# AI4Science-WestlakeU/wdno

Measured on AMD Instinct MI355X. Metric: diffusion train steps/sec, 2D smoke U-Net (8 samples per GPU per step), higher is better.
Workload: dtype f32

## Files before the change

include/wdno_hip.h:

```cpp
#ifndef WDNO_HIP_H
#define WDNO_HIP_H
#include <stdint.h>
#include <stddef.h>

#ifdef __cplusplus
extern "C" {
#endif

typedef void* wdno_stream_t;

enum { WDNO_OK = 0, WDNO_EINVAL = -1, WDNO_ELAUNCH = -2, WDNO_EUNSUPPORTED = -3, WDNO_EWORKSPACE = -4 };

#define WDNO_AMAX_SLOTS 64
#define WDNO_AMAX_STRIDE 16
#define WDNO_AMAX_FLOATS (WDNO_AMAX_SLOTS * WDNO_AMAX_STRIDE)
const char* wdno_strerror(int code);
int wdno_version(void);
const char* wdno_last_hip_error(void);
int wdno_set_debug(int mode);

typedef struct {
  int nd;
  int mode;
  int L;
  int n_img;
  int in_dims[3];
  int out_dims[3];
  int64_t cs_img, cs_band, cs0, cs1;
} wdno_dwt_desc;
size_t wdno_dwt_ws_bytes(const wdno_dwt_desc* d);
int wdno_dwt_fwd(const float* x, float* coef, const wdno_dwt_desc* d, const float* filters_host, void* ws, size_t ws_bytes, wdno_stream_t s);
int wdno_dwt_inv(const float* coef, float* x, const wdno_dwt_desc* d, const float* filters_host, void* ws, size_t ws_bytes, wdno_stream_t s);
int wdno_dwt_fwd_adjoint(const float* dcoef, float* dx, const wdno_dwt_desc* d, const float* filters_host, void* ws, size_t ws_bytes, wdno_stream_t s);
int wdno_dwt_inv_adjoint(const float* dx, float* dcoef, const wdno_dwt_desc* d, const float* filters_host, void* ws, size_t ws_bytes, wdno_stream_t s);
int wdno_dwt_fwd_packed(const float* x, float* state, const wdno_dwt_desc* d, const float* filters_host, int img_inner, int64_t cs_outer, int row_w,
                        const float* rescaler, wdno_stream_t s);
int wdno_upsample_coef(const float* in, float* out, int64_t outer, int a, int mid, int b, int c, int fa, int fb, int fc, wdno_stream_t s);
int wdno_pack_smoke_state(const float* coef, int64_t coef_sim_stride, const float* init_coef, int64_t init_sim_stride, const float* smokeout,
                          int64_t so_sim_stride, const int64_t* idx, const float* rescaler, float* state, int64_t B, int F, int nt, int nx,
                          int pad_t, int pad_x, wdno_stream_t s);
int wdno_pack_smoke_fields(const float* coef, int64_t coef_sim_stride, const float* rho0, int64_t rho0_sim_stride, const float* curve,
                           int64_t curve_sim_stride, const float* dec_lo_host, const float* dec_hi_host, int L, const float* rescaler,
                           float* state, int64_t B, int F, int nt, int nx, int pad_t, int pad_x, int H0, int W0, int T0, wdno_stream_t s);

int wdno_nc_to_cl(const float* src, float* dst, int64_t N, int C, int64_t S, int Cp, wdno_stream_t s);
int wdno_cl_to_nc(const float* src, float* dst, int64_t N, int C, int64_t S, int Cp, wdno_stream_t s);
int wdno_concat2_cl_planes(const float* a, int Ca, const float* b, int Cb, const float* rec_a, const float* rec_b, void* hi, void* lo,
                           float* scale_out, int64_t P, wdno_stream_t s);
int wdno_concat2_cl(const float* a, int Ca, const float* b, int Cb, float* out, int64_t P, wdno_stream_t s);
int wdno_concat2_cl_amax(const float* a, int Ca, const float* b, int Cb, float* out, float* amax_rec, int64_t P, wdno_stream_t s);
int wdno_split2_cl(const float* in, float* a, int Ca, float* b, int Cb, int64_t P, wdno_stream_t s);
int wdno_upsample2x_cl_fwd(const float* in, float* out, int64_t N, int H, int W, int C, wdno_stream_t s);
int wdno_upsample2x_cl_bwd(const float* dout, float* din, int64_t N, int H, int W, int C, wdno_stream_t s);

typedef struct {
  int N, D, H, W, C;
  int OD, OH, OW, K;
  int kd, kh, kw;
  int sd, sh, sw;
  int pd, ph, pw;
  int YD, YH, YW;
  int osd, osh, osw, ood, ooh, oow;
} wdno_conv_geom;
int wdno_conv_fwd(const float* x, const float* wp, const float* bias, const float* residual, float* y,
                  const wdno_conv_geom* g, wdno_stream_t s);
int wdno_amax(const float* x, int64_t n, float* amax_zeroed, wdno_stream_t s);
int wdno_amax_record(const float* x, int64_t n, float* rec_zeroed, wdno_stream_t s);
int wdno_split_f16(const float* x, const float* amax_rec, void* hi, void* lo, float* scale_out, int64_t rows, int C, int C8, wdno_stream_t s);
size_t wdno_split_colsum_ws_bytes(int64_t rows, int C8);
int wdno_split_f16_colsum(const float* x, const float* amax_rec, void* hi, void* lo, float* scale_out, float* colsum_out,
                          void* ws, size_t ws_bytes, int64_t rows, int C, int C8, wdno_stream_t s);
int wdno_pack_split_weight(const float* w, const float* amax, void* hi, void* lo, float* scale_out, int K, int C, int kd, int kh, int kw,
                           int A, int B, int mode, wdno_stream_t s);
typedef struct { const void* x; int64_t n; void* out; } wdno_amax_item;
typedef struct {
  const void* w; const void* amax; void* hi; void* lo; void* scale_out;
  int K, C, kd, kh, kw, A, B, mode;
} wdno_wsplit_item;
int wdno_amax_multi(const void* table, int n_items, int blocks_per_item, wdno_stream_t s);
int wdno_pack_split_weight_multi(const void* table, int n_items, int blocks_per_item, wdno_stream_t s);
int wdno_conv_fwd_f16x3(const void* xh, const void* xl, const float* sx, const void* wph, const void* wpl, const float* sw,
                        const float* bias, const float* residual, float* y, const wdno_conv_geom* g, wdno_stream_t s);
int wdno_conv_fwd_f16x3_amax(const void* xh, const void* xl, const float* sx, const void* wph, const void* wpl, const float* sw,
                             const float* bias, const float* residual, float* y, float* amax_rec, const wdno_conv_geom* g,
                             wdno_stream_t s);
typedef struct { int channels, d0, h0, w0; } wdno_zero_box;
int wdno_conv_fwd_f16x3_zbox(const void* xh, const void* xl, const float* sx, const void* wph, const void* wpl, const float* sw,
                             const float* bias, const float* residual, float* y, float* amax_rec, const wdno_conv_geom* g,
                             const wdno_zero_box* zb, wdno_stream_t s);
int wdno_conv_fwd_bf16_ex(const void* x16, const void* wp16, const float* bias, const float* residual, void* y, int y_bf16, float* amax_rec,
                          const wdno_conv_geom* g, const wdno_zero_box* zb, wdno_stream_t s);
int wdno_conv_fwd_f16x3_ws(const void* xh, const void* xl, const float* sx, const void* wph, const void* wpl, const float* sw,
                           const float* bias, const float* residual, float* y, float* amax_rec, const wdno_conv_geom* g,
                           void* ws, size_t ws_bytes, wdno_stream_t s);
size_t wdno_conv_fwd_split_ws_bytes(const wdno_conv_geom* g);
size_t wdno_conv_wgrad_f16x3_ws_bytes(const wdno_conv_geom* g);
int wdno_conv_pixel_table(void* table, const wdno_conv_geom* g, wdno_stream_t s);
int wdno_conv_wgrad_f16x3(const void* xh, const void* xl, const float* sx, const void* dyh, const void* dyl, const float* sdy,
                          const void* pixel_table, float* dwp, void* ws, size_t ws_bytes, const wdno_conv_geom* g, wdno_stream_t s);
int wdno_conv_wgrad_f16x3_param(const void* xh, const void* xl, const float* sx, const void* dyh, const void* dyl, const float* sdy,
                                const void* pixel_table, float* dw, int Kn, int Cn, void* ws, size_t ws_bytes,
                                const wdno_conv_geom* g, wdno_stream_t s);
#define WDNO_WGRAD_REDUCE_MAX 40
typedef struct wdno_wgrad_reduce_item {
  const float* ws; float* dw;
  int n, splits;
  int K8, C8, kw, ntap, Kn, Cn;
  int tiled;
  int reserved;
} wdno_wgrad_reduce_item;
int wdno_conv_wgrad_partials(const void* xh, const void* xl, const float* sx, const void* dyh, const void* dyl, const float* sdy,
                             const void* pixel_table, float* dw, int Kn, int Cn, void* ws, size_t ws_bytes,
                             const wdno_conv_geom* g, wdno_wgrad_reduce_item* item, wdno_stream_t s);
int wdno_wgrad_reduce_multi(const wdno_wgrad_reduce_item* items, int n_items, wdno_stream_t s);
size_t wdno_conv_wgrad_ws_bytes(const wdno_conv_geom* g);
int wdno_conv_wgrad(const float* x, const float* dy, float* dwp, void* ws, size_t ws_bytes,
                    const wdno_conv_geom* g, wdno_stream_t s);
#define WDNO_ROWS_SUM_MAX 64
typedef struct wdno_rows_sum_item {
  const void* part; float* out;
  int rows, stride, col0, ncols;
  int is_double, reserved;
} wdno_rows_sum_item;
int wdno_rows_sum_multi(const wdno_rows_sum_item* items, int n_items, wdno_stream_t s);
size_t wdno_colsum_ws_bytes(int64_t P, int C);
int wdno_colsum(const float* in, float* out, int64_t P, int C, void* ws, size_t ws_bytes, wdno_stream_t s);

int wdno_cast_bf16(const float* x, void* out16, int64_t rows, int C, int C8, wdno_stream_t s);
int wdno_cast_bf16_colsum(const float* x, void* out16, float* colsum_out, void* ws, size_t ws_bytes, int64_t rows, int C, int C8, wdno_stream_t s);
int wdno_conv_fwd_bf16(const void* x16, const void* wp16, const float* bias, const float* residual, float* y, float* amax_rec,
                       const wdno_conv_geom* g, wdno_stream_t s);
int wdno_conv_wgrad_bf16_param(const void* x16, const void* dy16, const void* pixel_table, float* dw, int Kn, int Cn, void* ws,
                               size_t ws_bytes, const wdno_conv_geom* g, wdno_stream_t s);

size_t wdno_groupnorm_ws_bytes(int64_t N, int64_t S, int C, int G);
size_t wdno_groupnorm_stats_floats(int64_t N, int C, int G);
int wdno_groupnorm_act_fwd(const float* x, const float* gamma, const float* beta, const float* ss, float* y,
                           float* stats, int64_t N, int64_t S, int C, int G, float eps, int silu,
                           void* ws, size_t ws_bytes, wdno_stream_t s);
int wdno_groupnorm_act_fwd_amax(const float* x, const float* gamma, const float* beta, const float* ss, float* y,
                                float* stats, float* amax_rec, int64_t N, int64_t S, int C, int G, float eps, int silu,
                                void* ws, size_t ws_bytes, wdno_stream_t s);
int wdno_groupnorm_act_bwd(const float* x, const float* dy, const float* gamma, const float* beta, const float* ss,
                           const float* stats, float* dx, float* dgb_partial, float* dss,
                           int64_t N, int64_t S, int C, int G, int silu, void* ws, size_t ws_bytes, wdno_stream_t s);
int wdno_groupnorm_act_bwd_amax(const float* x, const float* dy, const float* gamma, const float* beta, const float* ss,
                                const float* stats, float* dx, float* dgb_partial, float* dss, float* amax_rec,
                                int64_t N, int64_t S, int C, int G, int silu, void* ws, size_t ws_bytes, wdno_stream_t s);
size_t wdno_groupnorm_bwd_planes_ws_bytes(int64_t N, int64_t S, int C, int G);
size_t wdno_groupnorm_fwd_planes_ws_bytes(int64_t N, int64_t S, int C, int G);
int wdno_groupnorm_act_fwd_planes(const float* x, const float* gamma, const float* beta, const float* ss, void* y_hi, void* y_lo,
                                  float* y_scale, float* stats, float* bound_rec, int64_t N, int64_t S, int C, int G, float eps, int silu,
                                  void* ws, size_t ws_bytes, wdno_stream_t s);
int wdno_groupnorm_act_add_fwd_planes(const float* x, const float* gamma, const float* beta, const float* ss, const float* residual,
                                      const float* res_rec, float* y, void* y_hi, void* y_lo, float* y_scale, float* stats,
                                      float* bound_rec, float* y_amax_rec, int64_t N, int64_t S, int C, int G, float eps, int silu,
                                      void* ws, size_t ws_bytes, wdno_stream_t s);
int wdno_groupnorm_act_bwd_planes(const float* x, const float* dy, const float* gamma, const float* beta, const float* ss,
                                  const float* stats, void* dx_hi, void* dx_lo, float* dx_scale, float* dx_colsum,
                                  float* dgb_partial, float* dgb_sum, float* dss, float* bound_rec, int64_t N, int64_t S, int C, int G, int silu,
                                  void* ws, size_t ws_bytes, wdno_stream_t s);
int wdno_groupnorm_bwd_planes_tail(int64_t N, int64_t S, int C, int G, size_t* csp_offset, int* rows);
int wdno_groupnorm_act_fwd_amax_t(const void* x, int x_bf16, const float* gamma, const float* beta, const float* ss, float* y,
                                  float* stats, float* amax_rec, int64_t N, int64_t S, int C, int G, float eps, int silu,
                                  void* ws, size_t ws_bytes, wdno_stream_t s);
int wdno_groupnorm_act_fwd_planes_t(const void* x, int x_bf16, const float* gamma, const float* beta, const float* ss, void* y_hi, void* y_lo,
                                    float* y_scale, float* stats, float* bound_rec, int64_t N, int64_t S, int C, int G, float eps,
                                    int silu, void* ws, size_t ws_bytes, wdno_stream_t s);
int wdno_groupnorm_act_add_fwd_planes_t(const void* x, int x_bf16, const float* gamma, const float* beta, const float* ss, const float* residual,
                                        const float* res_rec, float* y, void* y_hi, void* y_lo, float* y_scale, float* stats,
                                        float* bound_rec, float* y_amax_rec, int64_t N, int64_t S, int C, int G, float eps, int silu,
                                        void* ws, size_t ws_bytes, wdno_stream_t s);
int wdno_groupnorm_act_bwd_planes_t(const void* x, int x_bf16, const void* dy, int dy_bf16, const float* gamma, const float* beta, const float* ss,
                                    const float* stats, void* dx_hi, void* dx_lo, float* dx_scale, float* dx_colsum,
                                    float* dgb_partial, float* dgb_sum, float* dss, float* bound_rec, int64_t N, int64_t S, int C, int G, int silu,
                                    void* ws, size_t ws_bytes, wdno_stream_t s);
int wdno_layernorm_fwd(const float* x, const float* g, float* y, int64_t P, int C, float eps, wdno_stream_t s);
int wdno_layernorm_fwd_amax(const float* x, const float* g, float* y, float* amax_rec, int64_t P, int C, float eps, wdno_stream_t s);
// ... 193 lines not shown
```

wdno_amd/_lib.py:

```python
import contextlib
import ctypes as C
import os

import torch

HERE = os.path.dirname(os.path.abspath(__file__))
LIB_PATH = os.path.join(HERE, 'libwdno_hip.so')

P = C.c_void_p
I = C.c_int
L = C.c_int64
F = C.c_float
Z = C.c_size_t


class DwtDesc(C.Structure):
    _fields_ = [('nd', I), ('mode', I), ('L', I), ('n_img', I), ('in_dims', I * 3), ('out_dims', I * 3),
                ('cs_img', L), ('cs_band', L), ('cs0', L), ('cs1', L)]


class ConvGeom(C.Structure):
    _fields_ = [(k, I) for k in ('N', 'D', 'H', 'W', 'C', 'OD', 'OH', 'OW', 'K', 'kd', 'kh', 'kw', 'sd', 'sh', 'sw',
                                 'pd', 'ph', 'pw', 'YD', 'YH', 'YW', 'osd', 'osh', 'osw', 'ood', 'ooh', 'oow')]

# ... 9 lines not shown

class WgradReduceItem(C.Structure):
    _fields_ = [('ws', C.c_void_p), ('dw', C.c_void_p), ('n', I), ('splits', I), ('K8', I), ('C8', I), ('kw', I), ('ntap', I), ('Kn', I), ('Cn', I),
                ('tiled', I), ('reserved', I)]


class RowsSumItem(C.Structure):
    _fields_ = [('part', C.c_void_p), ('out', C.c_void_p), ('rows', I), ('stride', I), ('col0', I), ('ncols', I), ('is_double', I), ('reserved', I)]


class BurgersDesc(C.Structure):
    _fields_ = [(k, I) for k in ('N', 's', 'nx0', 'nt_f', 'nxf', 'steps', 'record_time', 'f_time', 'num_t', 'sub_s', 'out_cols', 'waves',
                                 'points')] + [(k, F) for k in ('c', 'd', 'dm', 'dt')]


class BurgersGenerateDesc(C.Structure):
    _fields_ = [(k, I) for k in ('N', 's', 't', 'steps', 'record_time', 'f_time', 'num_t', 'st', 'sx', 'f_rows', 'cols', 'waves', 'points',
                                 'clamp')] + [(k, F) for k in ('c', 'd', 'dm', 'dt', 'alpha')]


class BurgersGuidanceDesc(C.Structure):
    _fields_ = [(k, I) for k in ('B', 'C', 'H', 'W', 'sample_stride', 'chan_stride', 'row_stride', 'h', 'w', 'n_t', 'n_x', 'L', 'mode', 'ntile',
                                 'tw', 'lds_bytes', 'num_timesteps', 'condition_f', 'clip_x0')] + [(k, F) for k in ('wu', 'wf')]


class SmokeSolveDesc(C.Structure):
    _fields_ = [(k, I) for k in ('B', 'nt', 'nx', 'time_interval', 'space_interval', 'num_t', 'max_iter', 'n_out', 'threads')] + [('accuracy', F)]


class SmokeGenerateDesc(C.Structure):
    _fields_ = [(k, I) for k in ('B', 'scenelength', 'record_scale', 'stride', 'max_iter', 'threads', 'noise_mode')] + [('accuracy', F), ('seed', C.c_uint64)]


PD, PG, PA, PC = C.POINTER(DwtDesc), C.POINTER(ConvGeom), C.POINTER(AttnDesc), C.POINTER(CondDesc)
PF = C.POINTER(C.c_float)

PROTOTYPES = {
    'wdno_strerror': (C.c_char_p, [I]),
    'wdno_version': (I, []),
    'wdno_last_hip_error': (C.c_char_p, []),
    'wdno_set_debug': (I, [I]),
    'wdno_dwt_ws_bytes': (Z, [PD]),
    'wdno_dwt_fwd': (I, [P, P, PD, PF, P, Z, P]),
    'wdno_dwt_fwd_packed': (I, [P, P, PD, PF, I, L, I, P, P]),
    'wdno_dwt_inv': (I, [P, P, PD, PF, P, Z, P]),
    'wdno_dwt_fwd_adjoint': (I, [P, P, PD, PF, P, Z, P]),
    'wdno_dwt_inv_adjoint': (I, [P, P, PD, PF, P, Z, P]),
    'wdno_upsample_coef': (I, [P, P, L, I, I, I, I, I, I, I, P]),
    'wdno_pack_smoke_state': (I, [P, L, P, L, P, L, P, P, P, L, I, I, I, I, I, P]),
    'wdno_pack_smoke_fields': (I, [P, L, P, L, P, L, PF, PF, I, P, P, L, I, I, I, I, I, I, I, I, P]),
    'wdno_nc_to_cl': (I, [P, P, L, I, L, I, P]),
    'wdno_cl_to_nc': (I, [P, P, L, I, L, I, P]),
    'wdno_concat2_cl': (I, [P, I, P, I, P, L, P]),
    'wdno_concat2_cl_planes': (I, [P, I, P, I, P, P, P, P, P, L, P]),
    'wdno_concat2_cl_amax': (I, [P, I, P, I, P, P, L, P]),
    'wdno_split2_cl': (I, [P, P, I, P, I, L, P]),
    'wdno_upsample2x_cl_fwd': (I, [P, P, L, I, I, I, P]),
    'wdno_upsample2x_cl_bwd': (I, [P, P, L, I, I, I, P]),
    'wdno_conv_fwd': (I, [P, P, P, P, P, PG, P]),
    'wdno_amax': (I, [P, L, P, P]),
    'wdno_amax_record': (I, [P, L, P, P]),
    'wdno_split_f16': (I, [P, P, P, P, P, L, I, I, P]),
    'wdno_split_colsum_ws_bytes': (Z, [L, I]),
    'wdno_split_f16_colsum': (I, [P, P, P, P, P, P, P, Z, L, I, I, P]),
    'wdno_pack_split_weight': (I, [P, P, P, P, P, I, I, I, I, I, I, I, I, P]),
    'wdno_amax_multi': (I, [P, I, I, P]),
    'wdno_pack_split_weight_multi': (I, [P, I, I, P]),
    'wdno_conv_fwd_f16x3': (I, [P, P, P, P, P, P, P, P, P, PG, P]),
    'wdno_conv_fwd_f16x3_amax': (I, [P, P, P, P, P, P, P, P, P, P, PG, P]),
    'wdno_conv_fwd_f16x3_ws': (I, [P, P, P, P, P, P, P, P, P, P, PG, P, Z, P]),
    'wdno_conv_fwd_split_ws_bytes': (Z, [PG]),
    'wdno_conv_wgrad_f16x3_ws_bytes': (Z, [PG]),
    'wdno_conv_pixel_table': (I, [P, PG, P]),
    'wdno_conv_wgrad_f16x3': (I, [P, P, P, P, P, P, P, P, P, Z, PG, P]),
    'wdno_conv_wgrad_f16x3_param': (I, [P, P, P, P, P, P, P, P, I, I, P, Z, PG, P]),
    'wdno_conv_wgrad_partials': (I, [P, P, P, P, P, P, P, P, I, I, P, Z, PG, P, P]),
    'wdno_wgrad_reduce_multi': (I, [P, I, P]),
    'wdno_rows_sum_multi': (I, [P, I, P]),
    'wdno_cast_bf16': (I, [P, P, L, I, I, P]),
    'wdno_cast_bf16_colsum': (I, [P, P, P, P, Z, L, I, I, P]),
    'wdno_conv_fwd_bf16': (I, [P, P, P, P, P, P, PG, P]),
    'wdno_conv_fwd_f16x3_zbox': (I, [P, P, P, P, P, P, P, P, P, P, PG, P, P]),
    'wdno_conv_fwd_bf16_ex': (I, [P, P, P, P, P, I, P, PG, P, P]),
    'wdno_conv_wgrad_bf16_param': (I, [P, P, P, P, I, I, P, Z, PG, P]),
    'wdno_conv_wgrad_ws_bytes': (Z, [PG]),
    'wdno_conv_wgrad': (I, [P, P, P, P, Z, PG, P]),
    'wdno_colsum_ws_bytes': (Z, [L, I]),
    'wdno_colsum': (I, [P, P, L, I, P, Z, P]),
    'wdno_groupnorm_ws_bytes': (Z, [L, L, I, I]),
    'wdno_groupnorm_stats_floats': (Z, [L, I, I]),
    'wdno_groupnorm_act_fwd': (I, [P, P, P, P, P, P, L, L, I, I, F, I, P, Z, P]),
    'wdno_groupnorm_act_fwd_amax': (I, [P, P, P, P, P, P, P, L, L, I, I, F, I, P, Z, P]),
    'wdno_groupnorm_act_bwd': (I, [P, P, P, P, P, P, P, P, P, L, L, I, I, I, P, Z, P]),
    'wdno_groupnorm_act_bwd_amax': (I, [P, P, P, P, P, P, P, P, P, P, L, L, I, I, I, P, Z, P]),
    'wdno_groupnorm_bwd_planes_ws_bytes': (Z, [L, L, I, I]),
    'wdno_groupnorm_bwd_planes_tail': (I, [L, L, I, I, C.POINTER(Z), C.POINTER(I)]),
    'wdno_groupnorm_fwd_planes_ws_bytes': (Z, [L, L, I, I]),
    'wdno_groupnorm_act_fwd_planes': (I, [P, P, P, P, P, P, P, P, P, L, L, I, I, F, I, P, Z, P]),
    'wdno_groupnorm_act_add_fwd_planes': (I, [P, P, P, P, P, P, P, P, P, P, P, P, P, L, L, I, I, F, I, P, Z, P]),
    'wdno_layernorm_fwd_planes': (I, [P, P, P, P, P, L, I, F, P]),
    'wdno_groupnorm_act_bwd_planes': (I, [P, P, P, P, P, P, P, P, P, P, P, P, P, P, L, L, I, I, I, P, Z, P]),
    'wdno_groupnorm_act_fwd_amax_t': (I, [P, I, P, P, P, P, P, P, L, L, I, I, F, I, P, Z, P]),
    'wdno_groupnorm_act_fwd_planes_t': (I, [P, I, P, P, P, P, P, P, P, P, L, L, I, I, F, I, P, Z, P]),
    'wdno_groupnorm_act_add_fwd_planes_t': (I, [P, I, P, P, P, P, P, P, P, P, P, P, P, P, L, L, I, I, F, I, P, Z, P]),
    'wdno_groupnorm_act_bwd_planes_t': (I, [P, I, P, I, P, P, P, P, P, P, P, P, P, P, P, P, L, L, I, I, I, P, Z, P]),
    'wdno_layernorm_fwd': (I, [P, P, P, L, I, F, P]),
    'wdno_layernorm_fwd_amax': (I, [P, P, P, P, L, I, F, P]),
    'wdno_layernorm_bwd_ws_bytes': (Z, [L, I]),
    'wdno_layernorm_bwd': (I, [P, P, P, P, P, L, I, F, P, Z, P]),
    'wdno_layernorm_bwd_add': (I, [P, P, P, P, P, P, L, I, F, P, Z, P]),
    'wdno_layernorm_bwd_add_amax': (I, [P, P, P, P, P, P, P, L, I, F, P, Z, P]),
    'wdno_attn_fwd': (I, [P, P, P, P, P, PA, F, P]),
    'wdno_attn_bwd_ws_bytes': (Z, [PA]),
    'wdno_attn_bwd': (I, [P, P, P, P, P, P, P, P, PA, F, P, Z, P]),
    'wdno_attn_fwd_amax': (I, [P, P, P, P, P, P, PA, F, P]),
    'wdno_attn_bwd_amax': (I, [P, P, P, P, P, P, P, P, P, PA, F, P, Z, P]),
    'wdno_attn_fwd_planes': (I, [P, P, P, P, P, P, P, P, P, P, PA, F, P]),
    'wdno_linattn_fwd_planes': (I, [P, P, P, P, P, P, P, L, I, I, F, P]),
    'wdno_attn_bwd_planes': (I, [P, P, P, P, P, P, P, P, P, P, P, P, PA, F, P, Z, P]),
    'wdno_tattn_fused_takes': (I, [I, I, I]),
    'wdno_tattn_fused_fwd': (I, [P, P, F, P, P, P, P, P, P, P, P, P, P, P, P, P, L, I, L, I, I, F, P]),
    'wdno_lattn_fused_takes': (I, [I, I, I]),
    'wdno_lattn_fused_ws_bytes': (Z, [L, I]),
    'wdno_lattn_fused_fwd': (I, [P, P, F, P, P, P, P, P, P, P, P, P, P, P, P, Z, L, I, I, I, F, P]),
    'wdno_lattn_fused_bwd_grads': (I, []),
    'wdno_lattn_fused_bwd_ws_bytes': (Z, [L, I]),
    'wdno_lattn_fused_bwd': (I, [P, P, P, F, P, P, P, P, P, P, P, P, P, P, P, P, P, Z, L, I, I, I, F, P]),
    'wdno_tattn_fused_bwd_ws_bytes': (Z, []),
    'wdno_tattn_fused_bwd_grads': (I, []),
    'wdno_tattn_fused_bwd': (I, [P, P, P, F, P, P, P, P, P, P, P, P, P, P, P, P, P, P, P, Z, L, I, L, I, I, F, P]),
    'wdno_linattn_ws_bytes': (Z, [L, I]),
    'wdno_linattn_fwd': (I, [P, P, P, P, L, I, I, F, P]),
    'wdno_linattn_bwd': (I, [P, P, P, P, P, P, Z, L, I, I, F, P]),
    'wdno_linattn_fwd_amax': (I, [P, P, P, P, P, L, I, I, F, P]),
    'wdno_linattn_bwd_amax': (I, [P, P, P, P, P, P, P, Z, L, I, I, F, P]),
    'wdno_linattn_bwd_planes': (I, [P, P, P, P, P, P, P, P, P, P, P, Z, L, I, I, F, P]),
    'wdno_act_fwd': (I, [P, P, L, I, P]),
    'wdno_act_bwd': (I, [P, P, P, L, I, P]),
    'wdno_linear_rows_fwd': (I, [P, I, P, I, P, P, I, I, I, I, P]),
    'wdno_linear_rows_wgrad': (I, [P, I, P, I, P, P, I, I, I, P]),
    'wdno_linear_multi_fwd': (I, [P, I, I, P, P, I, I, P]),
    'wdno_linear_multi_wgrad': (I, [P, I, I, P, P, P, P, I, I, P]),
    'wdno_linear_multi_dgrad_ws_bytes': (Z, [I, I, I]),
    'wdno_linear_multi_dgrad': (I, [P, I, I, P, P, I, I, P, Z, P]),
    'wdno_add': (I, [P, P, P, L, P]),
    'wdno_add_amax': (I, [P, P, P, P, L, P]),
    'wdno_sinusoidal_emb': (I, [P, P, P, I, I, P]),
    'wdno_q_sample_cond': (I, [P, P, P, P, P, P, P, PC, P]),
    'wdno_apply_cond': (I, [P, P, PC, P]),
    'wdno_weighted_mse_ws_bytes': (Z, [L]),
    'wdno_weighted_mse': (I, [P, P, P, P, F, P, P, L, L, I, L, P, Z, P]),
    'wdno_weighted_mse_bwd': (I, [P, P, P, P, F, P, P, L, L, I, L, P]),
    'wdno_p_sample_update': (I, [P, P, P, P, P, P, P, P, P, P, P, L, L, I, P]),
    'wdno_ddim_update': (I, [P, P, P, P, P, P, F, F, F, P, P, L, L, P]),
    'wdno_ddim_update_dev': (I, [P, P, P, P, P, P, P, P, P, L, L, P]),
    'wdno_sumsq_ws_bytes': (Z, [L]),
    'wdno_sumsq': (I, [P, L, P, P, Z, P]),
    'wdno_adam_clip_step': (I, [P, P, P, P, L, P, F, F, F, F, F, F, I, P]),
    'wdno_ema_update': (I, [P, P, L, F, P]),
    'wdno_gather_items': (I, [P, I, I, P]),
    'wdno_relpos_bias_fwd': (I, [P, P, P, I, I, P]),
    'wdno_relpos_bias_bwd': (I, [P, P, P, I, I, I, P]),
    'wdno_burgers_solve': (I, [P, P, P, C.POINTER(BurgersDesc), P]),
    'wdno_burgers_generate': (I, [P, P, P, P, P, C.POINTER(BurgersGenerateDesc), P]),
    'wdno_burgers_guidance': (I, [P, P, P, P, P, P, P, P, P, C.POINTER(BurgersGuidanceDesc), PF, P]),
    'wdno_smoke_solve': (I, [P, P, P, P, P, P, P, P, P, P, P, P, P, P, C.POINTER(SmokeSolveDesc), P]),
# ... 46 lines not shown
```

wdno_amd/csrc/conv_common.h:

```cpp
#pragma once
#include "common.h"

typedef float f32x16 __attribute__((ext_vector_type(16)));

#define BK 32
#define LDS_STRIDE 36

struct ConvP {
  wdno_conv_geom g;
  int R;
  int nchunk;
  int nsteps;
  int64_t P;
  int identity_out;
  int debug;
  int tiles_n;
  int ntiles;
  int ksplit;
  float* amax_rec;
  int tsplit;
  float* split_ws;
  size_t split_ws_bytes;
  int zb_blocks, zb_d, zb_h;
  int out_bf16;
};

__device__ __forceinline__ int xcd_swizzle(int bid, int nwg) {
  int q = nwg >> 3, r = nwg & 7;
  int xcd = bid & 7, idx = bid >> 3;
  int start = xcd < r ? xcd * (q + 1) : r * (q + 1) + (xcd - r) * q;
  return start + idx;
}

__device__ __forceinline__ int64_t out_row(const wdno_conv_geom& g, int64_t p) {
  int ow = (int)(p % g.OW); int64_t t = p / g.OW;
  int oh = (int)(t % g.OH); t /= g.OH;
  int od = (int)(t % g.OD);
  int64_t n = t / g.OD;
  return ((n * g.YD + (od * g.osd + g.ood)) * g.YH + (oh * g.osh + g.ooh)) * g.YW + (ow * g.osw + g.oow);
}

static inline int check_geom(const wdno_conv_geom* g) {
  if (!g) return WDNO_EINVAL;
  if (g->N <= 0 || g->D <= 0 || g->H <= 0 || g->W <= 0 || g->C <= 0 || g->K <= 0) return WDNO_EINVAL;
  if (g->OD <= 0 || g->OH <= 0 || g->OW <= 0 || g->kd <= 0 || g->kh <= 0 || g->kw <= 0) return WDNO_EINVAL;
  if (g->sd <= 0 || g->sh <= 0 || g->sw <= 0 || g->osd <= 0 || g->osh <= 0 || g->osw <= 0) return WDNO_EINVAL;
  if ((g->C & 3) || (g->K & 3)) return WDNO_EUNSUPPORTED;
  if ((g->OD - 1) * g->osd + g->ood >= g->YD || (g->OH - 1) * g->osh + g->ooh >= g->YH || (g->OW - 1) * g->osw + g->oow >= g->YW)
    return WDNO_EINVAL;
  return WDNO_OK;
}
#include "debug_modes.h"
void wdno_wgrad_h3d_plan(const wdno_conv_geom* g, int* bm, int* bn, int* splits, int* pix_per_split, int* splitpair = nullptr);
int wdno_conv_wgrad_h3_dma(const void* xh, const void* xl, const void* dyh, const void* dyl, const float* sx, const float* sdy,
                           const void* table, float* wsf, const wdno_conv_geom* g, hipStream_t st);
int wdno_conv_fwd_h3_dma(const void* xh, const void* xl, const void* wh, const void* wl, const float* sx, const float* sw,
                         const float* bias, const float* residual, float* y, ConvP& p, hipStream_t st, int stages);
bool wdno_conv_h3t_takes(const wdno_conv_geom& g);
int wdno_conv_h3t_split(const wdno_conv_geom& g, int64_t P, int cus);
int wdno_conv_fwd_h3_tap(int shape, const void* xh, const void* xl, const void* wh, const void* wl, const float* sx, const float* sw,
                         const float* bias, const float* residual, float* y, ConvP& p, hipStream_t st);
#ifdef __HIPCC__
__device__ __forceinline__ uint4 bf16x8_from_runs(float4 va, float4 vb) {
  const uint2 A = bf16x4_pack(va), B = bf16x4_pack(vb);
  const auto sx = __builtin_amdgcn_permlane32_swap(A.x, B.x, false, false);
  const auto sy = __builtin_amdgcn_permlane32_swap(A.y, B.y, false, false);
  return make_uint4(sx[0], sy[0], sx[1], sy[1]);
}
__device__ __forceinline__ void lgkm0_barrier() {
  __builtin_amdgcn_s_waitcnt(0xc07f);
  asm volatile("s_barrier" : : : "memory");
}
#endif
static inline void fill_params(ConvP& p, const wdno_conv_geom* g) {
  p.g = *g;
  p.amax_rec = nullptr;
  p.ksplit = 1;
  p.tsplit = 1;
  p.split_ws = nullptr;
  p.split_ws_bytes = 0;
  p.zb_blocks = 0; p.zb_d = 0; p.zb_h = 0;
  p.out_bf16 = 0;
  p.debug = wdno_debug_mode;
  p.R = g->kw * g->C;
  p.nchunk = cdiv(p.R, BK);
  p.nsteps = g->kd * g->kh * p.nchunk;
  p.P = (int64_t)g->N * g->OD * g->OH * g->OW;
  p.identity_out = (g->YD == g->OD && g->YH == g->OH && g->YW == g->OW && g->osd == 1 && g->osh == 1 && g->osw == 1 &&
                    g->ood == 0 && g->ooh == 0 && g->oow == 0) ? 1 : 0;
}
```

wdno_amd/csrc/conv_h3.hip:

```cpp
#include "conv_common.h"
#include <type_traits>
#include <algorithm>

typedef _Float16 half8 __attribute__((ext_vector_type(8)));
typedef __bf16 bf16x8 __attribute__((ext_vector_type(8)));
template <bool LP>
__device__ __forceinline__ f32x16 mfma_16(half8 a, half8 b, f32x16 c) {
  if constexpr (LP) return __builtin_amdgcn_mfma_f32_32x32x16_bf16(__builtin_bit_cast(bf16x8, a), __builtin_bit_cast(bf16x8, b), c, 0, 0, 0);
  else return __builtin_amdgcn_mfma_f32_32x32x16_f16(a, b, c, 0, 0, 0);
}

#define HBK 32
#define HST 40

template <bool RECORD>
__global__ __launch_bounds__(256) void amax_kernel(const float* __restrict__ x, int64_t n, unsigned* __restrict__ out) {
  __shared__ float red[4];
  const int64_t n4 = n >> 2;
  const float4* x4 = reinterpret_cast<const float4*>(x);
  float m = 0.f;
  const int64_t stride = (int64_t)gridDim.x * 1024;
  for (int64_t k0 = (int64_t)blockIdx.x * 1024 + threadIdx.x; k0 < n4; k0 += stride) {
    float4 v[4];
#pragma unroll
// ... 318 lines not shown
    _Float16* Bl = Bh + BN * HST;
#pragma unroll
    for (int i = 0; i < AROWS; ++i) {
      *reinterpret_cast<int4v*>(&Ah[(lrow + 64 * i) * HST + c8]) = ah[S][i];
      if (!LP) *reinterpret_cast<int4v*>(&Al[(lrow + 64 * i) * HST + c8]) = al[S][i];
    }
#pragma unroll
    for (int i = 0; i < BROWS; ++i) {
      *reinterpret_cast<int4v*>(&Bh[(lrow + 64 * i) * HST + c8]) = bh[S][i];
      if (!LP) *reinterpret_cast<int4v*>(&Bl[(lrow + 64 * i) * HST + c8]) = bl[S][i];
    }
  };

  const int wave = tid >> 6, lane = tid & 63;
  const int wm = wave / WN, wn = wave - wm * WN;
  const int li = lane & 31, hh = lane >> 5;
  const int m_base = wm * (TM * 32), n_base = wn * (TN * 32);

  f32x16 acc[TM][TN];
#pragma unroll
  for (int a = 0; a < TM; ++a)
#pragma unroll
    for (int b = 0; b < TN; ++b)
#pragma unroll
      for (int e = 0; e < 16; ++e) acc[a][b][e] = 0.f;

  using S0 = std::integral_constant<int, 0>;
  using S1 = std::integral_constant<int, 1>;
  auto iter = [&](auto PAR, int step) {
    constexpr int B = decltype(PAR)::value;
    const _Float16* Ah = hsm + B * STAGE;
    const _Float16* Al = Ah + BM * HST;
    const _Float16* Bh = Ah + NPL * BM * HST;
    const _Float16* Bl = Bh + BN * HST;
#pragma unroll
    for (int ks = 0; ks < 2; ++ks) {
      half8 fah[TM], fal[TM], fbh[TN], fbl[TN];
      const int col = ks * 16 + hh * 8;
#pragma unroll
      for (int a = 0; a < TM; ++a) {
        fah[a] = *reinterpret_cast<const half8*>(&Ah[(m_base + a * 32 + li) * HST + col]);
        if (!LP) fal[a] = *reinterpret_cast<const half8*>(&Al[(m_base + a * 32 + li) * HST + col]);
      }
#pragma unroll
      for (int b = 0; b < TN; ++b) {
        fbh[b] = *reinterpret_cast<const half8*>(&Bh[(n_base + b * 32 + li) * HST + col]);
        if (!LP) fbl[b] = *reinterpret_cast<const half8*>(&Bl[(n_base + b * 32 + li) * HST + col]);
      }
      if constexpr (!LP) {
#pragma unroll
        for (int a = 0; a < TM; ++a)
#pragma unroll
          for (int b = 0; b < TN; ++b) acc[a][b] = mfma_16<false>(fal[a], fbh[b], acc[a][b]);
#pragma unroll
        for (int a = 0; a < TM; ++a)
#pragma unroll
          for (int b = 0; b < TN; ++b) acc[a][b] = mfma_16<false>(fah[a], fbl[b], acc[a][b]);
      }
#pragma unroll
      for (int a = 0; a < TM; ++a)
#pragma unroll
        for (int b = 0; b < TN; ++b) acc[a][b] = mfma_16<LP>(fah[a], fbh[b], acc[a][b]);
    }
    using NXT = std::integral_constant<int, 1 - B>;
    if (step + 1 < nst) {
      wait_set(NXT{}, step + 2 < nst);
      store_tile(NXT{}, 1 - B);
    }
    __syncthreads();
    if (step + 3 < nst) load_tile(NXT{});
  };
  load_tile(S0{});
  wait_set(S0{}, false);
  store_tile(S0{}, 0);
  __syncthreads();
  if (nst > 1) load_tile(S1{});
  if (nst > 2) load_tile(S0{});
  for (int step = 0; step < nst; step += 2) {
    iter(S0{}, step);
    if (step + 1 < nst) iter(S1{}, step + 1);
  }

  const float inv = LP ? 1.0f : 1.0f / (sx[0] * sw[0]);
  float am = 0.f;
#pragma unroll
  for (int a = 0; a < TM; ++a) {
#pragma unroll
    for (int e = 0; e < 16; ++e) {
      int row = (e & 3) + 8 * (e >> 2) + 4 * hh;
      int64_t pm = m0 + m_base + a * 32 + row;
      if (pm >= p.P) continue;
      int64_t yr = p.identity_out ? pm : out_row(g, pm);
#pragma unroll
      for (int b = 0; b < TN; ++b) {
        int kc = n0 + n_base + b * 32 + li;
        if (kc < g.K) {
          float v = acc[a][b][e] * inv;
          if (p.ksplit > 1) {
            if (blockIdx.y == 0) {
              if (bias) v += bias[kc];
              if (res) v += res[yr * g.K + kc];
            }
            unsafeAtomicAdd(&y[yr * g.K + kc], v);
            continue;
          }
          if (bias) v += bias[kc];
          if (res) v += res[yr * g.K + kc];
          if (LP && p.out_bf16) reinterpret_cast<unsigned short*>(y)[yr * g.K + kc] = bf16_rne(v);
          else y[yr * g.K + kc] = v;
          am = fmaxf(am, fabsf(v));
        }
      }
    }
  }
  if (p.amax_rec) wave_amax_emit(am, p.amax_rec, (int)blockIdx.x * 4 + wave);
}

template <int BM, int BN, int WM, int WN, bool LP>
static int launch_h3(const void* xh, const void* xl, const void* wh, const void* wl, const float* sx, const float* sw,
                     const float* bias, const float* residual, float* y, ConvP& p, hipStream_t st) {
  const wdno_conv_geom& g = p.g;
  int64_t tiles_m = cdiv64(p.P, BM);
  p.tiles_n = cdiv(g.K, BN);
  int64_t nt = tiles_m * p.tiles_n;
  if (nt > 0x7fffffff) return WDNO_EUNSUPPORTED;
  p.ntiles = (int)nt;
  size_t lds = (size_t)2 * (LP ? 1 : 2) * (BM + BN) * HST * sizeof(_Float16);
  static bool attr_done = false;
  if (!attr_done) {
    (void)hipFuncSetAttribute((const void*)conv_fwd_h3_kernel<BM, BN, WM, WN, LP>, hipFuncAttributeMaxDynamicSharedMemorySize, (int)lds);
    attr_done = true;
  }
  const int64_t x_elems = (int64_t)g.N * g.D * g.H * g.W * g.C;
  const int64_t w_elems = (int64_t)g.kd * g.kh * g.K * p.R;
  if (x_elems * 2 >= OOB_OFFSET || w_elems * 2 >= OOB_OFFSET || p.P >= 0x7fffffff) return WDNO_EUNSUPPORTED;
  float* rec = p.amax_rec;
  if (p.ksplit > 1) {
    if (hipMemsetAsync(y, 0, (size_t)p.P * g.K * sizeof(float), st) != hipSuccess) return WDNO_ELAUNCH;
    p.amax_rec = nullptr;
  }
  conv_fwd_h3_kernel<BM, BN, WM, WN, LP><<<dim3((unsigned)p.ntiles, (unsigned)p.ksplit), 256, lds, st>>>(
      (const _Float16*)xh, (const _Float16*)xl, (const _Float16*)wh, (const _Float16*)wl, sx, sw, bias, residual, y, p,
      (unsigned)(x_elems * 2), (unsigned)(w_elems * 2));
  if (p.ksplit > 1 && rec) {
    amax_kernel<true><<<stream_grid(p.P * g.K / 16 + 1, 256), 256, 0, st>>>(y, p.P * g.K, reinterpret_cast<unsigned*>(rec));
    p.amax_rec = rec;
  }
  return WDNO_OK;
}

extern "C" int wdno_conv_fwd_f16x3(const void* xh, const void* xl, const float* sx, const void* wph, const void* wpl, const float* sw,
                                   const float* bias, const float* residual, float* y, const wdno_conv_geom* g, wdno_stream_t s) {
  return wdno_conv_fwd_f16x3_amax(xh, xl, sx, wph, wpl, sw, bias, residual, y, nullptr, g, s);
}
template <bool LP>
static int conv_fwd_16(const void* xh, const void* xl, const float* sx, const void* wph, const void* wpl, const float* sw,
                       const float* bias, const float* residual, float* y, float* amax_rec, const wdno_conv_geom* g, wdno_stream_t s,
                       float* split_ws = nullptr, size_t split_ws_bytes = 0, const wdno_zero_box* zb = nullptr, int y_bf16 = 0) {
  int rc = check_geom(g);
  if (rc) return rc;
  if (g->C & 7) return WDNO_EUNSUPPORTED;
  if (y_bf16 && (!LP || residual)) return WDNO_EUNSUPPORTED;
  ConvP p;
  fill_params(p, g);
  p.out_bf16 = y_bf16 ? 1 : 0;
  if (zb) {
    if (zb->channels < 0 || zb->d0 < 0 || zb->h0 < 0 || zb->w0 < 0) return WDNO_EINVAL;
    p.zb_blocks = zb->channels / 16; p.zb_d = zb->d0; p.zb_h = zb->h0;
  }
  p.amax_rec = amax_rec;
  p.split_ws = split_ws;
  p.split_ws_bytes = split_ws_bytes;
  p.nchunk = cdiv(p.R, HBK);
  p.nsteps = g->kd * g->kh * p.nchunk;
  hipStream_t st = as_stream(s);
  const int64_t P = p.P;
  const int K = g->K;
  auto blocks = [&](int bm, int bn) { return cdiv64(P, bm) * cdiv(K, bn); };
  const int dbg = wdno_debug_mode;
  const bool small_tap = p.identity_out && wdno_conv_h3t_takes(*g) && g->kw == 3 && blocks(64, 64) >= 64;
  if (dbg != WDNO_DBG_ROW_ATTN_AND_REG_STAGED_CONV && (dbg == WDNO_DBG_FORCE_DMA_CONV || dbg == WDNO_DBG_CHUNKED_DMA_CONV || dbg == WDNO_DBG_FORCE_TILES_160 || dbg == WDNO_DBG_FORCE_TILES_320 || small_tap || (K > 64 ? blocks(128, 128) : blocks(256, 64)) >= 100)) {
    rc = wdno_conv_fwd_h3_dma(xh, LP ? nullptr : xl, wph, LP ? nullptr : wpl, sx, sw, bias, residual, y, p, st, 3);
    if (rc == WDNO_OK) return wdno_check_launch();
    if (rc != WDNO_EUNSUPPORTED) return rc;
  }
  if (K > 64) {
    if (blocks(128, 128) >= 512 || blocks(64, 128) < 2 * blocks(128, 128)) rc = launch_h3<128, 128, 2, 2, LP>(xh, xl, wph, wpl, sx, sw, bias, residual, y, p, st);
    else if (blocks(64, 128) < 200) {
      if (blocks(64, 64) <= 384 && g->kd * g->kh >= 2 && p.nsteps >= 64 && p.identity_out && residual != y && !LP) p.ksplit = 2;
      rc = launch_h3<64, 64, 2, 2, LP>(xh, xl, wph, wpl, sx, sw, bias, residual, y, p, st);
    }
    else rc = launch_h3<64, 128, 1, 4, LP>(xh, xl, wph, wpl, sx, sw, bias, residual, y, p, st);
  } else {
    if (blocks(128, 64) >= 512 || P <= 128) rc = launch_h3<128, 64, 4, 1, LP>(xh, xl, wph, wpl, sx, sw, bias, residual, y, p, st);
    else rc = launch_h3<64, 64, 2, 2, LP>(xh, xl, wph, wpl, sx, sw, bias, residual, y, p, st);
  }
  if (rc) return rc;
  return wdno_check_launch();
}
extern "C" int wdno_conv_fwd_f16x3_amax(const void* xh, const void* xl, const float* sx, const void* wph, const void* wpl, const float* sw,
                                        const float* bias, const float* residual, float* y, float* amax_rec, const wdno_conv_geom* g,
                                        wdno_stream_t s) {
  return conv_fwd_16<false>(xh, xl, sx, wph, wpl, sw, bias, residual, y, amax_rec, g, s);
}
extern "C" int wdno_conv_fwd_f16x3_ws(const void* xh, const void* xl, const float* sx, const void* wph, const void* wpl, const float* sw,
                                      const float* bias, const float* residual, float* y, float* amax_rec, const wdno_conv_geom* g,
                                      void* ws, size_t ws_bytes, wdno_stream_t s) {
  return conv_fwd_16<false>(xh, xl, sx, wph, wpl, sw, bias, residual, y, amax_rec, g, s, (float*)ws, ws ? ws_bytes : 0);
}
extern "C" int wdno_conv_fwd_f16x3_zbox(const void* xh, const void* xl, const float* sx, const void* wph, const void* wpl, const float* sw,
                                        const float* bias, const float* residual, float* y, float* amax_rec, const wdno_conv_geom* g,
                                        const wdno_zero_box* zb, wdno_stream_t s) {
  return conv_fwd_16<false>(xh, xl, sx, wph, wpl, sw, bias, residual, y, amax_rec, g, s, nullptr, 0, zb);
}
extern "C" int wdno_conv_fwd_bf16_ex(const void* x16, const void* wp16, const float* bias, const float* residual, void* y, int y_bf16, float* amax_rec,
                                     const wdno_conv_geom* g, const wdno_zero_box* zb, wdno_stream_t s) {
  return conv_fwd_16<true>(x16, x16, nullptr, wp16, wp16, nullptr, bias, residual, (float*)y, amax_rec, g, s, nullptr, 0, zb, y_bf16);
}
extern "C" size_t wdno_conv_fwd_split_ws_bytes(const wdno_conv_geom* g) {
  if (!g || check_geom(g) || (g->C & 7)) return 0;
  ConvP p;
  fill_params(p, g);
  if (!p.identity_out || !wdno_conv_h3t_takes(*g)) return 0;
  const int runs = wdno_conv_h3t_split(*g, p.P, wdno_num_cus() & ~7);
  return runs > 1 ? (size_t)runs * p.P * g->K * sizeof(float) : 0;
}
extern "C" int wdno_conv_fwd_bf16(const void* x16, const void* wp16, const float* bias, const float* residual, float* y, float* amax_rec,
                                  const wdno_conv_geom* g, wdno_stream_t s) {
  return conv_fwd_16<true>(x16, x16, nullptr, wp16, wp16, nullptr, bias, residual, y, amax_rec, g, s);
}

typedef _Float16 half4 __attribute__((ext_vector_type(4)));
#define WH_BKP 32
#define WH_PAD 32

__global__ __launch_bounds__(256) void pixel_table_kernel(int4v* __restrict__ tbl, wdno_conv_geom g, int P) {
  int p = blockIdx.x * 256 + threadIdx.x;
  if (p >= P) return;
  int q = p;
  int ow = q % g.OW; q /= g.OW;
  int oh = q % g.OH; q /= g.OH;
  int od = q % g.OD;
  int n = q / g.OD;
  int d0 = od * g.sd - g.pd, h0 = oh * g.sh - g.ph, w0 = ow * g.sw - g.pw;
  int4v e;
  e.x = ((n * g.YD + (od * g.osd + g.ood)) * g.YH + (oh * g.osh + g.ooh)) * g.YW + (ow * g.osw + g.oow);
  e.y = (((n * g.D + d0) * g.H + h0) * g.W + w0) * g.C;
  e.z = (d0 << 16) | (h0 & 0xffff);
  e.w = w0;
  tbl[p] = e;
}
extern "C" int wdno_conv_pixel_table(void* table, const wdno_conv_geom* g, wdno_stream_t s) {
  int rc = check_geom(g);
  if (rc) return rc;
  int64_t P = (int64_t)g->N * g->OD * g->OH * g->OW;
  if (P >= 0x7fffffff || (int64_t)g->N * g->D * g->H * g->W * g->C >= 0x3fffffff) return WDNO_EUNSUPPORTED;
  pixel_table_kernel<<<(unsigned)cdiv64(P, 256), 256, 0, as_stream(s)>>>((int4v*)table, *g, (int)P);
  return wdno_check_launch();
}

struct WgradHP {
  ConvP c;
  int tiles_k, tiles_r, splits, bn;
  int64_t pix_per_split;
  int xcd_group;
};

__device__ __forceinline__ half8 tr_frag(const _Float16* tile, int stride, int pix0, int ch0, int lane) {
  const int g = lane >> 4, xl = lane & 15;
  const _Float16* p0 = tile + (pix0 + 8 * (g >> 1) + (xl >> 2)) * stride + ch0 + 16 * (g & 1) + 4 * (xl & 3);
  typedef short short4v __attribute__((ext_vector_type(4)));
  typedef short4v __attribute__((address_space(3))) * lds_s4;
  short4v a = __builtin_amdgcn_ds_read_tr16_b64_v4i16((lds_s4)(p0));
  short4v b = __builtin_amdgcn_ds_read_tr16_b64_v4i16((lds_s4)(p0 + 4 * stride));
  typedef short short8v __attribute__((ext_vector_type(8)));
  short8v c = __builtin_shufflevector(a, b, 0, 1, 2, 3, 4, 5, 6, 7);
  return __builtin_bit_cast(half8, c);
}

#define WH_RING 4
template <int BM, int BN, int WM, int WN, bool LP>
__global__ __launch_bounds__(256) void conv_wgrad_h3_kernel(const _Float16* __restrict__ xh, const _Float16* __restrict__ xl,
                                                             const _Float16* __restrict__ dyh, const _Float16* __restrict__ dyl,
                                                             const float* __restrict__ sx, const float* __restrict__ sdy,
                                                             const int4v* __restrict__ table, float* __restrict__ ws, WgradHP wpz,
                                                             unsigned x_bytes, unsigned dy_bytes) {
  constexpr int TM = BM / (WM * 32);
  constexpr int TN = BN / (WN * 32);
  constexpr int SA = BM + WH_PAD, SB = BN + WH_PAD;
  constexpr int A_C8 = BM / 8, B_C8 = BN / 8;
  constexpr int A_RPP = 256 / A_C8;
  constexpr int A_PASSES = WH_BKP / A_RPP, B_PASSES = WH_BKP * B_C8 / 256;
  static_assert(256 % A_C8 == 0 && (WH_BKP * B_C8) % 256 == 0, "loader mapping");
  constexpr int NPL = LP ? 1 : 2;
  constexpr int STAGE = NPL * WH_BKP * (SA + SB);
  extern __shared__ __attribute__((aligned(16))) _Float16 hsm[];
  int4v* pinfo = reinterpret_cast<int4v*>(hsm + 2 * STAGE);

  const ConvP& p = wpz.c;
  const wdno_conv_geom& g = p.g;
// ... 618 lines not shown
```

wdno_amd/csrc/conv_h3d.hip:

```cpp
#include "conv_common.h"
#include <type_traits>

typedef _Float16 half8 __attribute__((ext_vector_type(8)));
typedef __bf16 bf16x8 __attribute__((ext_vector_type(8)));
typedef int int4v __attribute__((ext_vector_type(4)));
#define DMA_OOB 0x7ffffff0
template <bool LP>
__device__ __forceinline__ f32x16 mfma_16(half8 a, half8 b, f32x16 c) {
  if constexpr (LP) return __builtin_amdgcn_mfma_f32_32x32x16_bf16(__builtin_bit_cast(bf16x8, a), __builtin_bit_cast(bf16x8, b), c, 0, 0, 0);
  else return __builtin_amdgcn_mfma_f32_32x32x16_f16(a, b, c, 0, 0, 0);
}

__device__ __forceinline__ int4v rsrc_words(const void* ptr, unsigned bytes) {
  uint64_t a = reinterpret_cast<uint64_t>(ptr);
  int4v r;
  r.x = __builtin_amdgcn_readfirstlane((int)(unsigned)a);
  r.y = __builtin_amdgcn_readfirstlane((int)(unsigned)((a >> 32) & 0xffffu));
  r.z = __builtin_amdgcn_readfirstlane((int)bytes);
  r.w = 0x00020000;
  return r;
}
__device__ __forceinline__ void dma_piece(int4v rsrc, int off, unsigned lds_dst) {
  asm volatile("s_mov_b32 m0, %1\n\ts_nop 0\n\tbuffer_load_dwordx4 %0, %2, 0 offen lds" : : "v"(off), "s"(lds_dst), "s"(rsrc) : "memory");
}
// ... 41 lines not shown
      int od = q % g.OD;
      int n = q / g.OD;
#pragma unroll
      for (int i = 0; i < AP; ++i) {
        const int d0 = od * g.sd - g.pd, h0 = oh * g.sh - g.ph, w0 = ow * g.sw - g.pw;
        a_off[i] = ((((n * g.D + d0) * g.H + h0) * g.W + w0) * g.C + c8) * 2;
        const unsigned m = tap_bits(d0, g.kd, g.D) | (tap_bits(h0, g.kh, g.H) << 8) | (tap_bits(w0, g.kw, g.W) << 16);
        a_mask[i] = (pm0 + 16 * i < p.P) ? m : 0u;
        ow += 16;
        while (ow >= g.OW) { ow -= g.OW; ++oh; }
        while (oh >= g.OH) { oh -= g.OH; ++od; }
        while (od >= g.OD) { od -= g.OD; ++n; }
      }
#pragma unroll
      for (int i = 0; i < BP; ++i) {
        const int k = tile_n * BN + pq * (BN / 4) + 16 * i + prow;
        b_ok[i] = k < g.K;
        b_off[i] = (k * p.R + c8) * 2;
      }
    };
    int c_tile = 0, s_chunk = 0, s_dz = 0, s_dy = 0, s_dx = 0, s_cc = 0;
    int x_uni = 0, w_uni = 0;
    int l_dx = c8 / g.C, l_cc = c8 % g.C;
    const int l_dx0 = l_dx, l_cc0 = l_cc;
    const int step_dx = 32 / g.C, step_cc = 32 % g.C;
    if (my_tiles > 0) setup_tile(0);
    const bool no_dma = p.debug == WDNO_DBG_NO_DMA || p.debug >= WDNO_DBG_NO_DMA_OFFSET;
    auto issue_step = [&](int stage) {
      const bool live = c_tile < my_tiles;
      const unsigned need_t = live ? ((1u << s_dz) | (1u << (8 + s_dy))) : 0x80000000u;
      const unsigned need = UNIFORM_DX ? (need_t | (1u << (16 + s_dx))) : (need_t | (1u << (16 + l_dx)));
      const unsigned pa_dst = lds0 + stage * STAGE + pq * (BM / 4) * 64, pb_dst = lds0 + stage * STAGE + B_HI + pq * (BN / 4) * 64;
#pragma unroll
      for (int i = 0; i < AP; ++i) {
        const int off = ((a_mask[i] & need) == need) ? a_off[i] + x_uni : DMA_OOB;
        if (no_dma) continue;
        dma_piece(rxh, off, pa_dst + i * 1024);
        if (!LP) dma_piece(rxl, off, pa_dst + A_LO + i * 1024);
      }
      const bool r_ok = live && (s_chunk * 32 + c8 < p.R);
#pragma unroll
      for (int i = 0; i < BP; ++i) {
        const int off = (b_ok[i] && r_ok) ? b_off[i] + w_uni : DMA_OOB;
        if (no_dma) continue;
        dma_piece(rwh, off, pb_dst + i * 1024);
        if (!LP) dma_piece(rwl, off, pb_dst + BN * 64 + i * 1024);
      }
      if (!live) return;
      ++s_chunk;
      x_uni += 64; w_uni += 64;
      if (UNIFORM_DX) {
        s_cc += 32;
        if (s_cc >= g.C) { s_cc = 0; ++s_dx; }
      } else {
        l_dx += step_dx; l_cc += step_cc;
        if (l_cc >= g.C) { l_cc -= g.C; ++l_dx; }
      }
      if (s_chunk == p.nchunk) {
        s_chunk = 0; s_dx = 0; s_cc = 0; l_dx = l_dx0; l_cc = l_cc0;
        if (++s_dy == g.kh) { s_dy = 0; ++s_dz; }
        if (s_dz == g.kd) {
          s_dz = 0;
          if (++c_tile < my_tiles) setup_tile(c_tile);
        }
        x_uni = (s_dz * g.H + s_dy) * g.W * g.C * 2;
        w_uni = (s_dz * g.kh + s_dy) * g.K * p.R * 2;
      }
    };
#pragma unroll
    for (int s = 0; s < NS - 1; ++s) issue_step(s);
    int stage = 0;
    const int total = my_tiles * p.nsteps;
    for (int gs = 0; gs < total; ++gs) {
      asm volatile("s_waitcnt vmcnt(%0)\n\ts_barrier" : : "n"((NS - 2) * PW) : "memory");
      int nstage = stage + NS - 1;
      if (nstage >= NS) nstage -= NS;
      issue_step(nstage);
      stage = stage + 1 == NS ? 0 : stage + 1;
    }
    asm volatile("s_waitcnt vmcnt(0)" : : : "memory");
    return;
  }

  float am = 0.f;
  const int wm = wave / WN, wn = wave - wm * WN;
  const int li = lane & 31, hh = lane >> 5;
  const int m_base = wm * (TM * 32), n_base = wn * (TN * 32);
  const int sw0 = (hh ^ ((li >> 2) & 3)) * 16;
  const int a_rd = (m_base + li) * 64 + sw0;
  const int b_rd = B_HI + (n_base + li) * 64 + sw0;
  half8 fah[2][TM], fal[2][TM], fbh[2][TN], fbl[2][TN];
  auto read_frags = [&](auto SET, int stage, int ks) {
    constexpr int B = decltype(SET)::value;
    const char* st = smem + stage * STAGE;
    const int x = ks * 32;
#pragma unroll
    for (int a = 0; a < TM; ++a) {
      fah[B][a] = *reinterpret_cast<const half8*>(st + ((a_rd + a * 2048) ^ x));
      if (!LP) fal[B][a] = *reinterpret_cast<const half8*>(st + A_LO + ((a_rd + a * 2048) ^ x));
    }
#pragma unroll
    for (int b = 0; b < TN; ++b) {
      fbh[B][b] = *reinterpret_cast<const half8*>(st + ((b_rd + b * 2048) ^ x));
      if (!LP) fbl[B][b] = *reinterpret_cast<const half8*>(st + BN * 64 + ((b_rd + b * 2048) ^ x));
    }
  };
  f32x16 acc[TM][TN];
  auto mfma_set = [&](auto SET) {
    constexpr int B = decltype(SET)::value;
    if constexpr (!LP) {
#pragma unroll
      for (int a = 0; a < TM; ++a)
#pragma unroll
        for (int b = 0; b < TN; ++b) acc[a][b] = mfma_16<false>(fbh[B][b], fal[B][a], acc[a][b]);
#pragma unroll
      for (int a = 0; a < TM; ++a)
#pragma unroll
        for (int b = 0; b < TN; ++b) acc[a][b] = mfma_16<false>(fbl[B][b], fah[B][a], acc[a][b]);
    }
#pragma unroll
    for (int a = 0; a < TM; ++a)
#pragma unroll
      for (int b = 0; b < TN; ++b) acc[a][b] = mfma_16<LP>(fbh[B][b], fah[B][a], acc[a][b]);
  };
  using B0 = std::integral_constant<int, 0>;
  using B1 = std::integral_constant<int, 1>;
  constexpr int NRD = NPL * (TM + TN), NMF = (LP ? 1 : 3) * TM * TN, RPM = (NRD + NMF - 1) / NMF;
  auto interleave = [&]() {
#pragma unroll
    for (int i = 0; i < NMF; ++i) {
      __builtin_amdgcn_sched_group_barrier(0x008, 1, 0);
      if (i * RPM < NRD) __builtin_amdgcn_sched_group_barrier(0x100, RPM, 0);
    }
  };
  const float inv = LP ? 1.0f : 1.0f / (sx[0] * sw[0]);
  int stage = 0;
  const int sdbg = p.debug >= WDNO_DBG_NO_DMA_OFFSET ? p.debug - WDNO_DBG_NO_DMA_OFFSET : p.debug;
  const bool stamps = sdbg == WDNO_DBG_STAMP_CYCLES || sdbg == WDNO_DBG_STAMP_EPILOGUE || sdbg == WDNO_DBG_STAMP_REALTIME;
  const uint64_t c_begin = stamps ? __builtin_amdgcn_s_memtime() : 0, r_begin = stamps ? __builtin_amdgcn_s_memrealtime() : 0;
  uint64_t c_epi = 0;
  for (int t = 0; t < my_tiles; ++t) {
    const int tile = xcd_swizzle((int)blockIdx.x + t * (int)gridDim.x, p.ntiles);
    const int tile_m = tile / p.tiles_n, tile_n = tile - tile_m * p.tiles_n;
    const int64_t m0 = (int64_t)tile_m * BM;
    const int n0 = tile_n * BN;
#pragma unroll
    for (int a = 0; a < TM; ++a)
#pragma unroll
      for (int b = 0; b < TN; ++b)
#pragma unroll
        for (int e = 0; e < 16; ++e) acc[a][b][e] = 0.f;
    lgkm0_barrier();
    read_frags(B0{}, stage, 0);
    for (int step = 0; step + 1 < p.nsteps; ++step) {
      read_frags(B1{}, stage, 1);
      mfma_set(B0{});
      interleave();
      __builtin_amdgcn_sched_barrier(0);
      stage = stage + 1 == NS ? 0 : stage + 1;
      lgkm0_barrier();
      read_frags(B0{}, stage, 0);
      mfma_set(B1{});
      interleave();
      __builtin_amdgcn_sched_barrier(0);
    }
    read_frags(B1{}, stage, 1);
    mfma_set(B0{});
    interleave();
    __builtin_amdgcn_sched_barrier(0);
    stage = stage + 1 == NS ? 0 : stage + 1;
    mfma_set(B1{});
    __builtin_amdgcn_sched_barrier(0);
    const uint64_t e_begin = stamps ? __builtin_amdgcn_s_memtime() : 0;
#pragma unroll
    for (int a = 0; a < TM; ++a) {
      const int64_t pm = m0 + m_base + a * 32 + li;
      if (pm >= p.P) continue;
      const int64_t yr = p.identity_out ? pm : out_row(g, pm);
      float* yrow = y + yr * g.K;
      const float* rrow = res ? res + yr * g.K : nullptr;
      if (LP && p.out_bf16) {
        unsigned short* y16 = reinterpret_cast<unsigned short*>(y) + yr * g.K;
#pragma unroll
        for (int b = 0; b < TN; ++b) {
#pragma unroll
          for (int e4 = 0; e4 < 4; e4 += 2) {
            const int k0 = n0 + n_base + b * 32 + 8 * e4;
            if (k0 >= g.K) continue;
            const int ka = k0 + 4 * hh, kb = ka + 8;
            float4 va = make_float4(acc[a][b][4 * e4] * inv, acc[a][b][4 * e4 + 1] * inv, acc[a][b][4 * e4 + 2] * inv, acc[a][b][4 * e4 + 3] * inv);
            float4 vb = make_float4(acc[a][b][4 * e4 + 4] * inv, acc[a][b][4 * e4 + 5] * inv, acc[a][b][4 * e4 + 6] * inv, acc[a][b][4 * e4 + 7] * inv);
            if (bias) {
              const float4 ta = *reinterpret_cast<const float4*>(bias + ka);
              va.x += ta.x; va.y += ta.y; va.z += ta.z; va.w += ta.w;
              if (k0 + 8 < g.K) { const float4 tb = *reinterpret_cast<const float4*>(bias + kb); vb.x += tb.x; vb.y += tb.y; vb.z += tb.z; vb.w += tb.w; }
            }
            const uint4 o = bf16x8_from_runs(va, vb);
            if (k0 + 8 * hh < g.K) *reinterpret_cast<uint4*>(y16 + k0 + 8 * hh) = o;
            am = amax4(amax4(am, va), vb);
          }
        }
        continue;
      }
#pragma unroll
      for (int b = 0; b < TN; ++b) {
#pragma unroll
        for (int e4 = 0; e4 < 4; ++e4) {
          const int kc = n0 + n_base + b * 32 + 8 * e4 + 4 * hh;
          if (kc < g.K) {
            float4 v = make_float4(acc[a][b][4 * e4] * inv, acc[a][b][4 * e4 + 1] * inv, acc[a][b][4 * e4 + 2] * inv, acc[a][b][4 * e4 + 3] * inv);
            if (bias) { const float4 t = *reinterpret_cast<const float4*>(bias + kc); v.x += t.x; v.y += t.y; v.z += t.z; v.w += t.w; }
            if (rrow) { const float4 t = *reinterpret_cast<const float4*>(rrow + kc); v.x += t.x; v.y += t.y; v.z += t.z; v.w += t.w; }
            *reinterpret_cast<float4*>(yrow + kc) = v;
            am = amax4(am, v);
          }
        }
      }
    }
    if (stamps) c_epi += __builtin_amdgcn_s_memtime() - e_begin;
  }
  if (stamps) am = sdbg == WDNO_DBG_STAMP_CYCLES ? (float)(__builtin_amdgcn_s_memtime() - c_begin) : sdbg == WDNO_DBG_STAMP_EPILOGUE ? (float)c_epi : (float)(__builtin_amdgcn_s_memrealtime() - r_begin);
  if (p.amax_rec) wave_amax_emit(am, p.amax_rec, (int)blockIdx.x * (WM * WN) + wave);
}

template <int BM, int BN, int WM, int WN, int NS, bool LP>
static int launch_h3d(const void* xh, const void* xl, const void* wh, const void* wl, const float* sx, const float* sw,
                      const float* bias, const float* residual, float* y, ConvP& p, hipStream_t st) {
  const wdno_conv_geom& g = p.g;
  int64_t tiles_m = cdiv64(p.P, BM);
  p.tiles_n = cdiv(g.K, BN);
  int64_t nt = tiles_m * p.tiles_n;
  if (nt > 0x7fffffff) return WDNO_EUNSUPPORTED;
  p.ntiles = (int)nt;
  const size_t lds = (size_t)NS * (LP ? 1 : 2) * (BM + BN) * 64;
  const int64_t x_elems = (int64_t)g.N * g.D * g.H * g.W * g.C;
  const int64_t w_elems = (int64_t)g.kd * g.kh * g.K * p.R;
  if (x_elems * 2 >= DMA_OOB || w_elems * 2 >= DMA_OOB || p.P >= 0x7fffffff) return WDNO_EUNSUPPORTED;
  int grid = wdno_num_cus() & ~7;
  if (grid < 8) grid = 8;
  if (p.ntiles < grid) grid = p.ntiles;
  const bool uni = (g.C % 32) == 0;
  if (uni) {
    static bool done = false;
    if (!done) { (void)hipFuncSetAttribute((const void*)conv_fwd_h3d_kernel<BM, BN, WM, WN, NS, true, LP>, hipFuncAttributeMaxDynamicSharedMemorySize, (int)lds); done = true; }
    conv_fwd_h3d_kernel<BM, BN, WM, WN, NS, true, LP><<<grid, 512, lds, st>>>((const _Float16*)xh, (const _Float16*)xl, (const _Float16*)wh, (const _Float16*)wl,
                                                                        sx, sw, bias, residual, y, p, (unsigned)(x_elems * 2), (unsigned)(w_elems * 2));
  } else {
    static bool done = false;
    if (!done) { (void)hipFuncSetAttribute((const void*)conv_fwd_h3d_kernel<BM, BN, WM, WN, NS, false, LP>, hipFuncAttributeMaxDynamicSharedMemorySize, (int)lds); done = true; }
    conv_fwd_h3d_kernel<BM, BN, WM, WN, NS, false, LP><<<grid, 512, lds, st>>>((const _Float16*)xh, (const _Float16*)xl, (const _Float16*)wh, (const _Float16*)wl,
                                                                         sx, sw, bias, residual, y, p, (unsigned)(x_elems * 2), (unsigned)(w_elems * 2));
  }
  return WDNO_OK;
}

template <bool LP>
static int fwd_h3_dma(const void* xh, const void* xl, const void* wh, const void* wl, const float* sx, const float* sw,
                      const float* bias, const float* residual, float* y, ConvP& p, hipStream_t st) {
  const wdno_conv_geom& g = p.g;
  if (g.kd > 8 || g.kh > 8 || g.kw > 8 || g.C < 8) return WDNO_EUNSUPPORTED;
  const int cus = wdno_num_cus() & ~7;
  auto cost = [&](int bm, int bn, double weight) {
    return (double)(cdiv64(cdiv64(p.P, bm) * cdiv(g.K, bn), cus) * bm * bn) * weight;
  };
  const bool narrow_only = g.K <= 64;
  int best = narrow_only ? 2 : 0;
  double c = narrow_only ? cost(256, 64, 1.04) : cost(128, 128, 1.0);
  if (!narrow_only && cost(192, 128, 1.0) < c) { best = 1; c = cost(192, 128, 1.0); }
  if (!narrow_only && cost(256, 64, 1.04) < c) { best = 2; c = cost(256, 64, 1.04); }
  if (cost(192, 64, 1.08) < c) { best = 3; c = cost(192, 64, 1.08); }
  if (p.identity_out && wdno_conv_h3t_takes(g)) {
    if (g.kw == 3) {
      if (!narrow_only && cost(160, 128, 1.02) < c) { best = 4; c = cost(160, 128, 1.02); }
      if (cost(320, 64, 1.05) < c) { best = 5; c = cost(320, 64, 1.05); }
      if (cost(128, 64, 1.15) < c) { best = 7; c = cost(128, 64, 1.15); }
      if (cost(64, 64, 1.35) < c) { best = 6; c = cost(64, 64, 1.35); }
      if (wdno_debug_mode == WDNO_DBG_FORCE_TILES_160) best = narrow_only ? 5 : 4;
      if (wdno_debug_mode == WDNO_DBG_FORCE_TILES_320) best = 5;
      const int split = wdno_conv_h3t_split(g, p.P, cus);
      if (best == 6 && split > 1 && p.split_ws && (size_t)split * p.P * g.K * sizeof(float) <= p.split_ws_bytes) { best = 0; p.tsplit = split; }
    }
    return wdno_conv_fwd_h3_tap(best, xh, LP ? nullptr : xl, wh, wl, sx, sw, bias, residual, y, p, st);
  }
  if (best == 0) return launch_h3d<128, 128, 2, 2, 3, LP>(xh, xl, wh, wl, sx, sw, bias, residual, y, p, st);
  if (best == 1) return launch_h3d<192, 128, 2, 2, 3, LP>(xh, xl, wh, wl, sx, sw, bias, residual, y, p, st);
  if (best == 3) return launch_h3d<192, 64, 2, 2, 3, LP>(xh, xl, wh, wl, sx, sw, bias, residual, y, p, st);
  return launch_h3d<256, 64, 4, 1, 3, LP>(xh, xl, wh, wl, sx, sw, bias, residual, y, p, st);
}
int wdno_conv_fwd_h3_dma(const void* xh, const void* xl, const void* wh, const void* wl, const float* sx, const float* sw,
                         const float* bias, const float* residual, float* y, ConvP& p, hipStream_t st, int stages) {
  (void)stages;
  if (xl == nullptr) return fwd_h3_dma<true>(xh, xh, wh, wh, sx, sw, bias, residual, y, p, st);
  return fwd_h3_dma<false>(xh, xl, wh, wl, sx, sw, bias, residual, y, p, st);
}
```

wdno_amd/csrc/conv_h3t.hip:

```cpp
#include "conv_common.h"
#include <type_traits>

typedef _Float16 half8 __attribute__((ext_vector_type(8)));
typedef __bf16 bf16x8 __attribute__((ext_vector_type(8)));
typedef int int4v __attribute__((ext_vector_type(4)));
#define T_OOB 0x7ffffff0

template <bool LP>
__device__ __forceinline__ f32x16 t_mfma(half8 a, half8 b, f32x16 c) {
  if constexpr (LP) return __builtin_amdgcn_mfma_f32_32x32x16_bf16(__builtin_bit_cast(bf16x8, a), __builtin_bit_cast(bf16x8, b), c, 0, 0, 0);
  else return __builtin_amdgcn_mfma_f32_32x32x16_f16(a, b, c, 0, 0, 0);
}
__device__ __forceinline__ int4v t_rsrc(const void* ptr, unsigned bytes) {
  uint64_t a = reinterpret_cast<uint64_t>(ptr);
  int4v r;
  r.x = __builtin_amdgcn_readfirstlane((int)(unsigned)a);
  r.y = __builtin_amdgcn_readfirstlane((int)(unsigned)((a >> 32) & 0xffffu));
  r.z = __builtin_amdgcn_readfirstlane((int)bytes);
  r.w = 0x00020000;
  return r;
}
__device__ __forceinline__ void t_piece(int4v rsrc, int off, unsigned lds_dst) {
  lds_dst = __builtin_amdgcn_readfirstlane(lds_dst);
  asm volatile("s_mov_b32 m0, %1\n\ts_nop 0\n\tbuffer_load_dwordx4 %0, %2, 0 offen lds" : : "v"(off), "s"(lds_dst), "s"(rsrc) : "memory");
// ... 136 lines not shown
    bool fresh = true;
    if (my_tiles > 0) setup_tile(0);
    const bool no_dma = p.debug == WDNO_DBG_NO_DMA || p.debug >= WDNO_DBG_NO_DMA_OFFSET;
    auto issue_stage = [&](int buf) {
      if (skipping) {
        if (fresh) {
          lv = tile_live(c_tile);
          s_dz = 0; s_dy = 0; s_cb = -1; s_cnt = 0; fresh = false;
          next_live();
        }
        x_uni = ((s_dz * g.H + s_dy) * g.W * g.C + s_cb * CB) * 2;
        w_uni = ((s_dz * g.kh + s_dy) * g.K * p.R + s_cb * CB) * 2;
      }
      const bool pad = s_dz == g.kd;
      const unsigned need = pad ? 0x10000u : (1u << s_dz) | (1u << (8 + s_dy));
      const unsigned dst = lds0 + buf * STAGE + pq * 1024;
#pragma unroll
      for (int i = 0; i < PA; ++i) {
        if (pq + 4 * i >= S::APIECES) continue;
        const int off = ((a_mask[i] & need) == need) ? a_off[i] + x_uni : T_OOB;
        if (no_dma) continue;
        t_piece(rxh, off, dst + i * 4096);
        if (!LP) t_piece(rxl, off, dst + A_LO + i * 4096);
      }
#pragma unroll
      for (int i = 0; i < PB; ++i) {
        if (pq + 4 * i >= S::BPIECES) continue;
        const int off = b_ok[i] && !pad ? b_off[i] + w_uni : T_OOB;
        if (no_dma) continue;
        t_piece(rwh, off, dst + B_HI + i * 4096);
        if (!LP) t_piece(rwl, off, dst + B_LO + i * 4096);
      }
      if (skipping) {
        ++s_cnt;
        if (!pad) next_live();
        if (s_dz >= g.kd && (pad || !(s_cnt & 1))) {
          fresh = true;
          if (++c_tile < my_tiles) setup_tile(c_tile);
        }
        return;
      }
      x_uni += ROWB; w_uni += ROWB;
      if constexpr (SP) {
        if (++s_cb == ncb) {
          s_cb = 0;
          if (++s_dy == g.kh) { s_dy = 0; ++s_dz; }
          x_uni = (s_dz * g.H + s_dy) * g.W * g.C * 2;
          w_uni = (s_dz * g.kh + s_dy) * g.K * p.R * 2;
        }
        if (--s_rem == 0 && ++c_tile < my_tiles) setup_tile(c_tile);
      } else if (pad || ++s_cb == ncb) {
        s_cb = 0;
        if (!pad && ++s_dy == g.kh) { s_dy = 0; ++s_dz; }
        if (s_dz == g.kd && (pad || !padded)) {
          s_dz = 0;
          if (++c_tile < my_tiles) setup_tile(c_tile);
        }
        x_uni = (s_dz * g.H + s_dy) * g.W * g.C * 2;
        w_uni = (s_dz * g.kh + s_dy) * g.K * p.R * 2;
      }
    };
    const int total = my_tiles * nstages;
    int buf = 0;
    if (skipping) {
      if (my_tiles > 0) issue_stage(0);
      for (int left = my_tiles > 0 ? 1 : 0; left > 0; --left) {
        asm volatile("s_waitcnt vmcnt(0)\n\ts_barrier" : : : "memory");
        buf ^= 1;
        if (c_tile < my_tiles) { issue_stage(buf); ++left; }
      }
      asm volatile("s_waitcnt vmcnt(0)" : : : "memory");
      return;
    }
    if (total > 0) issue_stage(0);
    for (int gs = 0; gs < total; ++gs) {
      asm volatile("s_waitcnt vmcnt(0)\n\ts_barrier" : : : "memory");
      buf ^= 1;
      if (gs + 1 < total) issue_stage(buf);
    }
    asm volatile("s_waitcnt vmcnt(0)" : : : "memory");
    return;
  }

  float am = 0.f;
  const int wm = wave / WN, wn = wave - wm * WN;
  const int li = lane & 31, hh = lane >> 5;
  const int m_base = wm * (TM * 32), n_base = wn * (TN * 32);
  const int b_row = n_base + li;
  auto swz = [](int row) { return CB == 32 ? ((row >> 2) & 3) : ((row >> 3) & 1); };
  const int b_rd = B_HI + b_row * ROWB + ((hh ^ swz(b_row)) * 16);
  int a_rd[TM][KW];
  half8 fah[2][TM], fal[2][TM], fbh[2][TN], fbl[2][TN];
  auto read_frags = [&](int set, int boff, int dx, int ks) {
    const char* st = smem + boff;
    const int x = ks * 32;
#pragma unroll
    for (int a = 0; a < TM; ++a) {
      fah[set][a] = *reinterpret_cast<const half8*>(st + (a_rd[a][dx] ^ x));
      if (!LP) fal[set][a] = *reinterpret_cast<const half8*>(st + A_LO + (a_rd[a][dx] ^ x));
    }
#pragma unroll
    for (int b = 0; b < TN; ++b) {
      fbh[set][b] = *reinterpret_cast<const half8*>(st + dx * (BN * ROWB) + b * (32 * ROWB) + (b_rd ^ x));
      if (!LP) fbl[set][b] = *reinterpret_cast<const half8*>(st + B_PLANE + dx * (BN * ROWB) + b * (32 * ROWB) + (b_rd ^ x));
    }
  };
  f32x16 acc[TM][TN];
  auto mfma_set = [&](int set) {
    if constexpr (!LP) {
#pragma unroll
      for (int a = 0; a < TM; ++a)
#pragma unroll
        for (int b = 0; b < TN; ++b) acc[a][b] = t_mfma<false>(fbh[set][b], fal[set][a], acc[a][b]);
#pragma unroll
      for (int a = 0; a < TM; ++a)
#pragma unroll
        for (int b = 0; b < TN; ++b) acc[a][b] = t_mfma<false>(fbl[set][b], fah[set][a], acc[a][b]);
    }
#pragma unroll
    for (int a = 0; a < TM; ++a)
#pragma unroll
      for (int b = 0; b < TN; ++b) acc[a][b] = t_mfma<LP>(fbh[set][b], fah[set][a], acc[a][b]);
  };
  const float inv = LP ? 1.0f : 1.0f / (sx[0] * sw[0]);
  const int sdbg = p.debug >= WDNO_DBG_NO_DMA_OFFSET ? p.debug - WDNO_DBG_NO_DMA_OFFSET : p.debug;
  const bool stamps = sdbg == WDNO_DBG_STAMP_CYCLES || sdbg == WDNO_DBG_STAMP_EPILOGUE || sdbg == WDNO_DBG_STAMP_REALTIME;
  const uint64_t c_begin = stamps ? __builtin_amdgcn_s_memtime() : 0, r_begin = stamps ? __builtin_amdgcn_s_memrealtime() : 0;
  uint64_t c_epi = 0;
  int boff = 0;
  for (int t = 0; t < my_tiles; ++t) {
    const int vt = xcd_swizzle((int)blockIdx.x + t * (int)gridDim.x, nvt);
    const int run = SP ? vt / p.ntiles : 0, tile = vt - run * p.ntiles;
    const int tile_m = tile / p.tiles_n, tile_n = tile - tile_m * p.tiles_n;
    const int64_t m0 = (int64_t)tile_m * BM;
    const int n0 = tile_n * BN;
    int row0 = m_base + li;
    asm volatile("" : "+v"(row0));
#pragma unroll
    for (int a = 0; a < TM; ++a) {
      const int ow = ((int)m0 + row0 + a * 32) % g.OW;
#pragma unroll
      for (int dx = 0; dx < KW; ++dx) {
        const int row = row0 + a * 32 + dx;
        const bool ok = (unsigned)(ow - g.pw + dx) < (unsigned)g.W;
        const int zrow = S::ZB + (row & (S::ZR - 1));
        a_rd[a][dx] = (ok ? row : zrow) * ROWB + ((hh ^ swz(row)) * 16);
      }
    }
#pragma unroll
    for (int a = 0; a < TM; ++a)
#pragma unroll
      for (int b = 0; b < TN; ++b)
#pragma unroll
        for (int e = 0; e < 16; ++e) asm volatile("v_mov_b32 %0, 0" : "=v"(acc[a][b][e]));
    lgkm0_barrier();
    read_frags(0, boff, 0, 0);
    constexpr int NRD = NPL * (TM + TN), NMF = (LP ? 1 : 3) * TM * TN;
    constexpr int RPM = (NRD + NMF - 1) / NMF;
    auto interleave = [&]() {
#pragma unroll
      for (int i = 0; i < NMF; ++i) {
        __builtin_amdgcn_sched_group_barrier(0x008, 1, 0);
        if (i * RPM < NRD) __builtin_amdgcn_sched_group_barrier(0x100, RPM, 0);
      }
    };
    auto stage_body = [&](auto PARC, auto LASTC) {
      constexpr int PAR = decltype(PARC)::value;
// ... 7 lines not shown
          lgkm0_barrier();
          read_frags((PAR + NSUB) & 1, boff, 0, 0);
        }
        mfma_set((PAR + sub) & 1);
        if (sub + 1 < NSUB || !LAST) interleave();
        __builtin_amdgcn_sched_barrier(0);
      }
    };
    using P0 = std::integral_constant<int, 0>;
    using P1 = std::integral_constant<int, 1>;
    if constexpr (NSUB % 2 == 0) {
      for (int s = 0; s + 1 < nstages; ++s) stage_body(P0{}, std::false_type{});
      stage_body(P0{}, std::true_type{});
    } else if constexpr (KW != 7) {
      for (int s = 0; s + 2 < nstages; s += 2) { stage_body(P0{}, std::false_type{}); stage_body(P1{}, std::false_type{}); }
      stage_body(P0{}, std::false_type{});
      stage_body(P1{}, std::true_type{});
    } else {
      const unsigned allz = (1u << g.kd) - 1u, ally = (1u << g.kh) - 1u;
      const TapLive lvc = skipping ? tile_live(t) : TapLive{{allz, allz}, {ally, ally}};
      const int nst = t_live_stages(lvc, ncb, nzb);
      f32x16 acc2[TM][TN];
#pragma unroll
      for (int a = 0; a < TM; ++a)
#pragma unroll
        for (int b = 0; b < TN; ++b)
#pragma unroll
          for (int e = 0; e < 16; ++e) asm volatile("v_mov_b32 %0, 0" : "=v"(acc2[a][b][e]));
      int g_dz = 0, g_dy = -1, flush_at = 0;
      auto next_row = [&]() {
        for (;;) {
          if (++g_dy == g.kh) { g_dy = 0; ++g_dz; }
          if (g_dz >= g.kd) { flush_at = 0x7fffffff; return; }
          const int n = (int)((lvc.z[0] >> g_dz) & (lvc.y[0] >> g_dy) & 1u) * nzb + (int)((lvc.z[1] >> g_dz) & (lvc.y[1] >> g_dy) & 1u) * (ncb - nzb);
          if (n) { flush_at += n; return; }
        }
      };
      next_row();
      auto row_done = [&](int done) {
        if (done != flush_at) return;
#pragma unroll
        for (int a = 0; a < TM; ++a)
#pragma unroll
          for (int b = 0; b < TN; ++b)
#pragma unroll
            for (int e = 0; e < 16; ++e) {
              acc2[a][b][e] += acc[a][b][e];
              asm volatile("v_mov_b32 %0, 0" : "=v"(acc[a][b][e]));
            }
        next_row();
      };
      for (int s = 0; s + 2 < nst; s += 2) {
        stage_body(P0{}, std::false_type{}); row_done(s + 1);
        stage_body(P1{}, std::false_type{}); row_done(s + 2);
      }
      stage_body(P0{}, std::false_type{}); row_done(nst - 1);
      stage_body(P1{}, std::true_type{});
#pragma unroll
      for (int a = 0; a < TM; ++a)
#pragma unroll
        for (int b = 0; b < TN; ++b)
#pragma unroll
          for (int e = 0; e < 16; ++e) acc[a][b][e] += acc2[a][b][e];
    }
    boff = STAGE - boff;
    const uint64_t e_begin = stamps ? __builtin_amdgcn_s_memtime() : 0;
#pragma unroll
    for (int a = 0; a < TM; ++a) {
      const int64_t pm = m0 + m_base + a * 32 + li;
      if (pm >= p.P) continue;
      const int64_t yr = pm;
      if constexpr (SP) {
        float* wrow = p.split_ws + ((int64_t)run * p.P + pm) * g.K;
#pragma unroll
        for (int b = 0; b < TN; ++b) {
#pragma unroll
          for (int e4 = 0; e4 < 4; ++e4) {
            const int kc = n0 + n_base + b * 32 + 8 * e4 + 4 * hh;
            if (kc < g.K) *reinterpret_cast<float4*>(wrow + kc) = make_float4(acc[a][b][4 * e4], acc[a][b][4 * e4 + 1], acc[a][b][4 * e4 + 2], acc[a][b][4 * e4 + 3]);
          }
        }
        continue;
      }
      float* yrow = y + yr * g.K;
      const float* rrow = res ? res + yr * g.K : nullptr;
      if (LP && p.out_bf16) {
        unsigned short* y16 = reinterpret_cast<unsigned short*>(y) + yr * g.K;
#pragma unroll
        for (int b = 0; b < TN; ++b) {
#pragma unroll
          for (int e4 = 0; e4 < 4; e4 += 2) {
            const int k0 = n0 + n_base + b * 32 + 8 * e4;
            if (k0 >= g.K) continue;
            const int ka = k0 + 4 * hh, kb = ka + 8;
            float4 va = make_float4(acc[a][b][4 * e4] * inv, acc[a][b][4 * e4 + 1] * inv, acc[a][b][4 * e4 + 2] * inv, acc[a][b][4 * e4 + 3] * inv);
            float4 vb = make_float4(acc[a][b][4 * e4 + 4] * inv, acc[a][b][4 * e4 + 5] * inv, acc[a][b][4 * e4 + 6] * inv, acc[a][b][4 * e4 + 7] * inv);
            if (bias) {
              const float4 ta = *reinterpret_cast<const float4*>(bias + ka);
              va.x += ta.x; va.y += ta.y; va.z += ta.z; va.w += ta.w;
              if (k0 + 8 < g.K) { const float4 tb = *reinterpret_cast<const float4*>(bias + kb); vb.x += tb.x; vb.y += tb.y; vb.z += tb.z; vb.w += tb.w; }
            }
            const uint4 o = bf16x8_from_runs(va, vb);
            if (k0 + 8 * hh < g.K) *reinterpret_cast<uint4*>(y16 + k0 + 8 * hh) = o;
            am = amax4(amax4(am, va), vb);
          }
        }
        continue;
      }
#pragma unroll
      for (int b = 0; b < TN; ++b) {
#pragma unroll
        for (int e4 = 0; e4 < 4; ++e4) {
          const int kc = n0 + n_base + b * 32 + 8 * e4 + 4 * hh;
          if (kc < g.K) {
            float4 v = make_float4(acc[a][b][4 * e4] * inv, acc[a][b][4 * e4 + 1] * inv, acc[a][b][4 * e4 + 2] * inv, acc[a][b][4 * e4 + 3] * inv);
            if (bias) { const float4 tb = *reinterpret_cast<const float4*>(bias + kc); v.x += tb.x; v.y += tb.y; v.z += tb.z; v.w += tb.w; }
            if (rrow) { const float4 tr = *reinterpret_cast<const float4*>(rrow + kc); v.x += tr.x; v.y += tr.y; v.z += tr.z; v.w += tr.w; }
            *reinterpret_cast<float4*>(yrow + kc) = v;
            am = amax4(am, v);
          }
        }
      }
    }
    if (stamps) c_epi += __builtin_amdgcn_s_memtime() - e_begin;
  }
  if (stamps) am = sdbg == WDNO_DBG_STAMP_CYCLES ? (float)(__builtin_amdgcn_s_memtime() - c_begin) : sdbg == WDNO_DBG_STAMP_EPILOGUE ? (float)c_epi : (float)(__builtin_amdgcn_s_memrealtime() - r_begin);
  if (p.amax_rec) wave_amax_emit(am, p.amax_rec, (int)blockIdx.x * (WM * WN) + wave);
}

__global__ __launch_bounds__(256) void conv_split_reduce_kernel(const float4* __restrict__ ws, int nruns, int64_t n4, int K4, const float* __restrict__ sx,
                                                                 const float* __restrict__ sw, const float4* __restrict__ bias, const float4* res,
                                                                 float4* y, float* __restrict__ amax_rec) {
  const float inv = sx ? 1.0f / (sx[0] * sw[0]) : 1.0f;
  float am = 0.f;
  for (int64_t i = (int64_t)blockIdx.x * 256 + threadIdx.x; i < n4; i += (int64_t)gridDim.x * 256) {
    float4 v = ws[i];
    for (int r = 1; r < nruns; ++r) { const float4 u = ws[(int64_t)r * n4 + i]; v.x += u.x; v.y += u.y; v.z += u.z; v.w += u.w; }
    v.x *= inv; v.y *= inv; v.z *= inv; v.w *= inv;
    if (bias) { const float4 tb = bias[(int)(i % K4)]; v.x += tb.x; v.y += tb.y; v.z += tb.z; v.w += tb.w; }
    if (res) { const float4 tr = res[i]; v.x += tr.x; v.y += tr.y; v.z += tr.z; v.w += tr.w; }
    y[i] = v;
    am = amax4(am, v);
  }
  if (amax_rec) wave_amax_emit(am, amax_rec, (int)blockIdx.x * 4 + (int)(threadIdx.x >> 6));
}

template <int BM, int BN, int WM, int WN, int KW, int CB, bool LP, bool SP = false>
static int launch_h3t(const void* xh, const void* xl, const void* wh, const void* wl, const float* sx, const float* sw,
                      const float* bias, const float* residual, float* y, ConvP& p, hipStream_t st) {
  using S = TapShape<BM, BN, KW, CB>;
  const wdno_conv_geom& g = p.g;
  int64_t tiles_m = cdiv64(p.P, BM);
  p.tiles_n = cdiv(g.K, BN);
  int64_t nt = tiles_m * p.tiles_n;
  if (nt > 0x7fffffff) return WDNO_EUNSUPPORTED;
  p.ntiles = (int)nt;
  constexpr size_t lds = (size_t)2 * (LP ? 1 : 2) * (S::A_PLANE + S::B_PLANE);
  static_assert(lds <= 160 * 1024, "two stages must fit the LDS");
  const int64_t x_elems = (int64_t)g.N * g.D * g.H * g.W * g.C;
  const int64_t w_elems = (int64_t)g.kd * g.kh * g.K * p.R;
  if (x_elems * 2 >= T_OOB || w_elems * 2 >= T_OOB || p.P >= 0x7fffffff - BM) return WDNO_EUNSUPPORTED;
  if (SP) {
    const int nst = g.kd * g.kh * ((g.C + CB - 1) / CB);
    if (p.tsplit < 2 || ((CB / 16) * KW & 1) || nst % p.tsplit || !p.split_ws || (size_t)p.tsplit * p.P * g.K * sizeof(float) > p.split_ws_bytes || (g.K & 3))
      return WDNO_EINVAL;
  } else p.tsplit = 1;
  int grid = wdno_num_cus() & ~7;
  if (grid < 8) grid = 8;
  if ((int64_t)p.ntiles * p.tsplit < grid) grid = p.ntiles * p.tsplit;
  static bool done = false;
  if (!done) { (void)hipFuncSetAttribute((const void*)conv_fwd_h3t_kernel<BM, BN, WM, WN, KW, CB, LP, SP>, hipFuncAttributeMaxDynamicSharedMemorySize, (int)lds); done = true; }
  conv_fwd_h3t_kernel<BM, BN, WM, WN, KW, CB, LP, SP><<<grid, 512, lds, st>>>((const _Float16*)xh, (const _Float16*)xl, (const _Float16*)wh, (const _Float16*)wl,
                                                                    sx, sw, bias, residual, y, p, (unsigned)(x_elems * 2), (unsigned)(w_elems * 2));
  if (p.tsplit > 1) {
    const int64_t n4 = p.P * g.K / 4;
    conv_split_reduce_kernel<<<(unsigned)std::min<int64_t>((n4 + 255) / 256, 2048), 256, 0, st>>>(
        (const float4*)p.split_ws, p.tsplit, n4, g.K / 4, LP ? nullptr : sx, sw, (const float4*)bias, (const float4*)residual, (float4*)y, p.amax_rec);
  }
  return WDNO_OK;
}

static bool t_stem(const wdno_conv_geom& g) { return g.kw == 7 && (g.C % 16) == 0 && g.K <= 64; }
bool wdno_conv_h3t_takes(const wdno_conv_geom& g) {
  return g.sd == 1 && g.sh == 1 && g.sw == 1 && g.OD == g.D && g.OH == g.H && g.OW == g.W && ((g.kw == 3 && (g.C % 32) == 0) || t_stem(g)) &&
         g.kd <= 8 && g.kh <= 8 && wdno_debug_mode != WDNO_DBG_CHUNKED_DMA_CONV;
}
int wdno_conv_h3t_split(const wdno_conv_geom& g, int64_t P, int cus) {
  if (wdno_debug_mode == WDNO_DBG_CONV_NO_RUN_SPLIT || g.kw != 3 || (g.C % 32) || g.K < 128 || (g.K & 3)) return 1;
  const int64_t t128 = cdiv64(P, 128) * cdiv(g.K, 128);
  const int nst = g.kd * g.kh * (g.C / 32);
  return t128 * 4 <= cus && nst % 4 == 0 && nst / 4 >= 8 ? 4 : 1;
}
template <bool LP>
static int fwd_h3t(int shape, const void* xh, const void* xl, const void* wh, const void* wl, const float* sx, const float* sw,
                   const float* bias, const float* residual, float* y, ConvP& p, hipStream_t st) {
  if (shape == 0 && p.tsplit > 1 && !LP) return launch_h3t<128, 128, 2, 2, 3, 32, false, true>(xh, xl, wh, wl, sx, sw, bias, residual, y, p, st);
  if (shape == 0) return launch_h3t<128, 128, 2, 2, 3, 32, LP>(xh, xl, wh, wl, sx, sw, bias, residual, y, p, st);
  if (shape == 1) return launch_h3t<192, 128, 2, 2, 3, 32, LP>(xh, xl, wh, wl, sx, sw, bias, residual, y, p, st);
  if (shape == 3) return launch_h3t<192, 64, 2, 2, 3, 32, LP>(xh, xl, wh, wl, sx, sw, bias, residual, y, p, st);
  if (shape == 4) return launch_h3t<160, 128, 1, 4, 3, 32, LP>(xh, xl, wh, wl, sx, sw, bias, residual, y, p, st);
  if (shape == 5) return launch_h3t<320, 64, 2, 2, 3, 32, LP>(xh, xl, wh, wl, sx, sw, bias, residual, y, p, st);
  if (shape == 6) return launch_h3t<64, 64, 2, 2, 3, 32, LP>(xh, xl, wh, wl, sx, sw, bias, residual, y, p, st);
  if (shape == 7) return launch_h3t<128, 64, 2, 2, 3, 32, LP>(xh, xl, wh, wl, sx, sw, bias, residual, y, p, st);
  return launch_h3t<256, 64, 4, 1, 3, 32, LP>(xh, xl, wh, wl, sx, sw, bias, residual, y, p, st);
}
int wdno_conv_fwd_h3_tap(int shape, const void* xh, const void* xl, const void* wh, const void* wl, const float* sx, const float* sw,
                         const float* bias, const float* residual, float* y, ConvP& p, hipStream_t st) {
  if (p.g.kw == 7) {
    const int ncb = (p.g.C + 15) / 16;
    if (p.zb_blocks >= ncb) p.zb_blocks = ncb - 1;
// ... 12 lines not shown
```

wdno_amd/ops.py:

```python
import contextlib
import ctypes as C
import math
import os

import torch

from . import _lib
from ._lib import AttnDesc, CondDesc, ConvGeom, DwtDesc

WEIGHT_EPOCH = 0
_pack_cache = {}


PROFILE = None


class _timed:

    def __init__(self, key, flops):
        self.key, self.flops = key, flops

    def __enter__(self):
        if PROFILE is not None:
            self.e0 = torch.cuda.Event(enable_timing=True)
# ... 50 lines not shown
    if not t.is_cuda:
        raise RuntimeError(f'wdno_amd: {name} must live on the GPU (no CPU fallback on the hot path)')
    if t.dtype != torch.float32:
        raise RuntimeError(f'wdno_amd: {name} must be float32, got {t.dtype}')
    return t if t.is_contiguous() else t.contiguous()


def _chk_act(t, name='tensor'):
    if t.dtype != torch.bfloat16:
        return _chk(t, name)
    if not t.is_cuda:
        raise RuntimeError(f'wdno_amd: {name} must live on the GPU (no CPU fallback on the hot path)')
    return t if t.is_contiguous() else t.contiguous()


def _ws(nbytes, device):
    return torch.empty(max(int(nbytes), 16), dtype=torch.uint8, device=device)


def pad4(c):
    return (c + 3) // 4 * 4


class _NcToCl(torch.autograd.Function):
    @staticmethod
    def forward(ctx, x, cp):
        x = _chk(x, 'x')
        n, c = x.shape[0], x.shape[1]
        sp = tuple(x.shape[2:])
        s = int(math.prod(sp))
        out = torch.empty((n, *sp, cp), device=x.device, dtype=torch.float32)
        _lib.check(_lib_().wdno_nc_to_cl(_p(x), _p(out), n, c, s, cp, _stream()), 'nc_to_cl')
        ctx.c = c
        return out

    @staticmethod
    def backward(ctx, g):
        return cl_to_nc_raw(_chk(g, 'grad'), ctx.c), None


def cl_to_nc_raw(x, c):
    n, cp = x.shape[0], x.shape[-1]
    sp = tuple(x.shape[1:-1])
    s = int(math.prod(sp))
    out = torch.empty((n, c, *sp), device=x.device, dtype=torch.float32)
    _lib.check(_lib_().wdno_cl_to_nc(_p(x), _p(out), n, c, s, cp, _stream()), 'cl_to_nc')
    return out


class _ClToNc(torch.autograd.Function):
    @staticmethod
    def forward(ctx, x, c):
        x = _chk(x, 'x')
        ctx.cp = x.shape[-1]
        return cl_to_nc_raw(x, c)

    @staticmethod
    def backward(ctx, g):
        g = _chk(g, 'grad')
        n, c = g.shape[0], g.shape[1]
        sp = tuple(g.shape[2:])
        out = torch.empty((n, *sp, ctx.cp), device=g.device, dtype=torch.float32)
        _lib.check(_lib_().wdno_nc_to_cl(_p(g), _p(out), n, c, int(math.prod(sp)), ctx.cp, _stream()), 'nc_to_cl')
        return out, None


def nc_to_cl(x, cp=None):
    return _NcToCl.apply(x, pad4(x.shape[1]) if cp is None else cp)


def cl_to_nc(x, c):
    return _ClToNc.apply(x, c)


class _Concat(torch.autograd.Function):
    @staticmethod
    def forward(ctx, a, b, planes_only=False):
        ra, rb = _known_amax(a), _known_amax(b)
        a, b = _chk(a, 'a'), _chk(b, 'b')
        ca, cb = a.shape[-1], b.shape[-1]
        p = a.numel() // ca
        out = torch.empty((*a.shape[:-1], ca + cb), device=a.device, dtype=torch.float32)
        ctx.ca, ctx.cb = ca, cb
        if (planes_only and PLANES_FWD and CONV_MATH in ('f16x3', 'bf16') and ca % 8 == 0 and cb % 8 == 0
                and (_lp() or (ra is not None and rb is not None))):
            hi = torch.empty((p, ca + cb), device=a.device, dtype=torch.float16)
            lo = sc = None
            if not _lp():
                lo = torch.empty((p, ca + cb), device=a.device, dtype=torch.float16)
                sc = torch.empty((1,), device=a.device, dtype=torch.float32)
            _lib.check(_lib_().wdno_concat2_cl_planes(_p(a), ca, _p(b), cb, _p(ra), _p(rb), _p(hi), _p(lo), _p(sc), p, _stream()), 'concat2_planes')
            return _planes_only(out, (hi, lo, sc))
        rec = _new_amax_record(a.device)
        _lib.check(_lib_().wdno_concat2_cl_amax(_p(a), ca, _p(b), cb, _p(out), _p(rec), p, _stream()), 'concat2_cl')
        return _leave_amax(out, rec)

    @staticmethod
    def backward(ctx, g):
        g = _chk(g, 'grad')
        ca, cb = ctx.ca, ctx.cb
        p = g.numel() // (ca + cb)
        ga = torch.empty((*g.shape[:-1], ca), device=g.device, dtype=torch.float32)
        gb = torch.empty((*g.shape[:-1], cb), device=g.device, dtype=torch.float32)
        _lib.check(_lib_().wdno_split2_cl(_p(g), _p(ga), ca, _p(gb), cb, p, _stream()), 'split2_cl')
        return ga, gb, None


def concat_cl(a, b, planes_only=False):
    return _Concat.apply(a, b, planes_only)


def resnet_reads_planes(x_pixels, block):
    rc = getattr(block, 'res_conv', None)
    return (rc is not None and hasattr(rc, 'weight') and conv_reads_planes(x_pixels, block.block1.proj.weight)
            and conv_reads_planes(x_pixels, rc.weight))


class _Up2x(torch.autograd.Function):
    @staticmethod
    def forward(ctx, x):
        x = _chk(x, 'x')
        n, h, w, c = x.shape
        out = torch.empty((n, 2 * h, 2 * w, c), device=x.device, dtype=torch.float32)
        _lib.check(_lib_().wdno_upsample2x_cl_fwd(_p(x), _p(out), n, h, w, c, _stream()), 'upsample2x_fwd')
        return out

    @staticmethod
    def backward(ctx, g):
        g = _chk(g, 'grad')
        n, h2, w2, c = g.shape
        out = torch.empty((n, h2 // 2, w2 // 2, c), device=g.device, dtype=torch.float32)
        _lib.check(_lib_().wdno_upsample2x_cl_bwd(_p(g), _p(out), n, h2 // 2, w2 // 2, c, _stream()), 'upsample2x_bwd')
        return out


def upsample2x_cl(x):
    return _Up2x.apply(x)


class _Act(torch.autograd.Function):
    @staticmethod
    def forward(ctx, x, kind):
        x = _chk(x, 'x')
        y = torch.empty_like(x)
        _lib.check(_lib_().wdno_act_fwd(_p(x), _p(y), x.numel(), kind, _stream()), 'act_fwd')
        ctx.save_for_backward(x)
        ctx.kind = kind
        return y

    @staticmethod
    def backward(ctx, g):
        (x,) = ctx.saved_tensors
        g = _chk(g, 'grad')
        dx = torch.empty_like(x)
        _lib.check(_lib_().wdno_act_bwd(_p(x), _p(g), _p(dx), x.numel(), ctx.kind, _stream()), 'act_bwd')
        return dx, None


def silu(x):
    return _Act.apply(x, 0)


def gelu(x):
    return _Act.apply(x, 1)


class _Add(torch.autograd.Function):
    @staticmethod
    def forward(ctx, a, b):
        a, b = _chk(a, 'a'), _chk(b, 'b')
        assert a.shape == b.shape
        out = torch.empty_like(a)
        rec = _new_amax_record(a.device)
        _lib.check(_lib_().wdno_add_amax(_p(a), _p(b), _p(out), _p(rec), a.numel(), _stream()), 'add')
        return _leave_amax(out, rec)

    @staticmethod
    def backward(ctx, g):
        return g, g


def add(a, b):
    return _Add.apply(a, b)


def silu_shared(t):
    h = getattr(t, '_wdno_silu', None)
    if h is not None and h[1] == t._version and h[2] == torch.is_grad_enabled():
        return h[0]
    a = silu(t)
    try:
        t._wdno_silu = (a, t._version, torch.is_grad_enabled())
    except Exception:
        pass
    return a


_freq_cache = {}


def sinusoidal_embedding(t, dim, theta=10000.0):
    t = t.to(torch.int64).contiguous()
    if not t.is_cuda:
        raise RuntimeError('wdno_amd: timesteps must live on the GPU')
    key = (dim, float(theta), str(t.device))
    if key not in _freq_cache:
        half = dim // 2
        _freq_cache[key] = torch.exp(torch.arange(half) * -(math.log(theta) / (half - 1))).to(torch.float32).to(t.device)
    out = torch.empty((t.shape[0], dim), device=t.device, dtype=torch.float32)
    _lib.check(_lib_().wdno_sinusoidal_emb(_p(t), _p(_freq_cache[key]), _p(out), t.shape[0], dim, _stream()), 'sinusoidal_emb')
    return out


def _geom(x_shape, c, k, ks, st, pd, out_sp, y_sp=None, ostride=(1, 1, 1), ooff=(0, 0, 0)):
    n, d, h, w = x_shape
    y_sp = out_sp if y_sp is None else y_sp
    return ConvGeom(n, d, h, w, c, out_sp[0], out_sp[1], out_sp[2], k, ks[0], ks[1], ks[2], st[0], st[1], st[2],
                    pd[0], pd[1], pd[2], y_sp[0], y_sp[1], y_sp[2], ostride[0], ostride[1], ostride[2],
                    ooff[0], ooff[1], ooff[2])


def _as5(w):
    if w.dim() == 2:
        return w[:, :, None, None, None]
    if w.dim() == 4:
        return w[:, :, None]
    return w


def _cached(w, kind, cp, kp, build):
    key = (w.data_ptr(), kind, cp, kp, tuple(w.shape), tuple(w.stride()))
    ver = (w._version, WEIGHT_EPOCH)
    hit = _pack_cache.get(key)
    if hit is not None and hit[0] == ver:
        return hit[1]
    with torch.no_grad():
        packed = build().contiguous()
    if len(_pack_cache) > 4096:
        _pack_cache.clear()
        bump_weight_epoch(params=False)
    _pack_cache[key] = (ver, packed, w.detach())
    return packed


def _padded(w5, kp, cp):
    k, c = w5.shape[0], w5.shape[1]
    if k == kp and c == cp:
        return w5
    out = w5.new_zeros((kp, cp, *w5.shape[2:]))
    out[:k, :c] = w5
    return out


def pack_fwd(w, cp, kp):
    return _cached(w, 'f', cp, kp, lambda: _padded(_as5(w.detach()), kp, cp).permute(2, 3, 0, 4, 1))


def pack_dgrad(w, cp, kp):
    return _cached(w, 'd', cp, kp, lambda: _padded(_as5(w.detach()), kp, cp).flip(2, 3, 4).permute(2, 3, 1, 4, 0))


def pack_transposed(w_io, cin_p, cout_p):
    def build():
        w = w_io.detach()
        cin, cout = w.shape[0], w.shape[1]
        out = w.new_zeros((2, 2, 1, 2, cout_p, 2, cin_p))
        for py in range(2):
            for px in range(2):
                for dy in range(2):
                    for dx in range(2):
                        out[py, px, 0, dy, :cout, dx, :cin] = w[:, :, 0, 3 - py - 2 * dy, 3 - px - 2 * dx].t()
        return out
    return _cached(w_io, 't', cin_p, cout_p, build)


CONV_MATH = os.environ.get('WDNO_CONV_MATH', 'f16x3')
LOWP_AVAILABLE = True


def _lp():
    return CONV_MATH == 'bf16'


@contextlib.contextmanager
def _math(mode):
    global CONV_MATH
    prev, CONV_MATH = CONV_MATH, mode
    try:
        yield
    finally:
        CONV_MATH = prev
H3_MIN_PIXELS = 1024
PATCH_DGRAD_H3 = True
H3_MIN_REDUCTION = 64


def pad8(c):
    return (c + 7) // 8 * 8


_amax_pool = {}
AMAX_FLOATS = 64 * 16
AMAX_HINTS = True


PLANES_FWD = True
GRAD_PLANES = True
_CAPTURE = None


@contextlib.contextmanager
def graph_capture(graph, stream=None):
    global _CAPTURE
    assert _CAPTURE is None, 'nested graph captures are not supported'
    with torch.cuda.graph(graph, stream=stream, capture_error_mode='thread_local'):
        _CAPTURE = [None, 0]
        try:
            yield graph
        finally:
            _CAPTURE = None


def _amax_slot(device):
    if _CAPTURE is not None:
        st = _CAPTURE
        if st[0] is None or st[1] >= st[0].shape[0]:
            st[0], st[1] = torch.zeros((1024, AMAX_FLOATS), device=device, dtype=torch.float32), 0
        rec = st[0][st[1]]
        st[1] += 1
        return rec
    key = str(device)
    st = _amax_pool.get(key)
    if st is None or st[1] >= st[0].shape[0]:
        st = [torch.zeros((1024, AMAX_FLOATS), device=device, dtype=torch.float32), 0]
        _amax_pool[key] = st
    rec = st[0][st[1]]
    st[1] += 1
    return rec


def _new_amax_record(device):
    return _amax_slot(device) if AMAX_HINTS and not _lp() else None


def _leave_amax(t, rec):
    if rec is not None:
        t._wdno_amax = (rec, t._version)
    return t


def _known_amax(t):
    h = getattr(t, '_wdno_amax', None)
    return h[0] if h is not None and h[1] == t._version and AMAX_HINTS else None


def tensor_amax(x):
    amax = _amax_slot(x.device)
    _lib.check(_lib_().wdno_amax_record(_p(x), x.numel(), _p(amax), _stream()), 'amax')
    return amax


def split_f16_of(t, x2d, amax=None, c8=None):
    h = getattr(t, '_wdno_planes', None)
    if (h is not None and h[1] == t._version and h[0][0].shape[0] == x2d.shape[0] and h[2] == CONV_MATH
            and (c8 is None or h[0][0].shape[1] == c8)):
        return h[0]
    planes = split_f16(x2d, amax, c8)
    try:
        t._wdno_planes = (planes, t._version, CONV_MATH)
    except Exception:
        pass
    return planes


def split_f16(x2d, amax=None, c8=None):
    rows, c = x2d.shape
    if c8 is None or _lp():
        c8 = pad8(c)
    lib = _lib_()
    if _lp():
        hi = torch.empty((rows, c8), device=x2d.device, dtype=torch.float16)
        _lib.check(lib.wdno_cast_bf16(_p(x2d), _p(hi), rows, c, c8, _stream()), 'cast_bf16')
        return hi, None, None
    if amax is None:
        amax = tensor_amax(x2d)
    hi = torch.empty((rows, c8), device=x2d.device, dtype=torch.float16)
    lo = torch.empty((rows, c8), device=x2d.device, dtype=torch.float16)
    scale = amax[1:2]
    _lib.check(lib.wdno_split_f16(_p(x2d), _p(amax), _p(hi), _p(lo), _p(scale), rows, c, c8, _stream()), 'split_f16')
    return hi, lo, scale
# ... 124 lines not shown
    return [pl for pl in _wplans.values() if since is None or pl.used >= since]


def touch_plans(plans):
    e = WEIGHT_EPOCH
    for pl in plans:
        pl.used = e


def prepare_graph_refresh():
    epoch = WEIGHT_EPOCH
    for pl in _wplans.values():
        if pl.used >= epoch - 3:
            pl.used = epoch
    bump_weight_epoch(params=False)
    if _wplans:
        for lp in {pl.lp for pl in _wplans.values()}:
            _refresh_weight_plans(WEIGHT_EPOCH, lp)
    bump_weight_epoch(params=False)


def split_weight(w, kind, cp8, kp, pack=None):
    lp = _lp()
    key = (w.data_ptr(), kind, cp8, kp, tuple(w.shape), tuple(w.stride()), lp)
    ver = (w._version, WEIGHT_EPOCH)
    pl = _wplans.get(key)
    if pl is not None:
        if pl.ver != ver:
            _refresh_weight_plans(WEIGHT_EPOCH)
        if pl.ver == ver:
            pl.used = WEIGHT_EPOCH
            return pl.hi, pl.lo, pl.sc
    with torch.no_grad():
        wd = w.detach()
        wc = wd if wd.is_contiguous() else wd.contiguous()
        amax = None
        if not lp:
            amax = torch.zeros(1, device=w.device, dtype=torch.float32)
            _lib.check(_lib_().wdno_amax(_p(wc), wc.numel(), _p(amax), _stream()), 'amax')
        k, c, kd, kh, kw = _wdims(kind, _as5(wc))
        rows = kd * kh * kp * kw
        if pl is None:
            pl = _WPlan()
            pl.w, pl.wd, pl.kind, pl.cp8, pl.kp, pl.lp = wd, wd, kind, cp8, kp, lp
            pl.hi = torch.empty((rows, cp8), device=w.device, dtype=torch.float16)
            pl.lo = None if lp else torch.empty((rows, cp8), device=w.device, dtype=torch.float16)
            pl.sc = None if lp else torch.empty(1, device=w.device, dtype=torch.float32)
            if len(_wplans) > 4096:
                _wplans.clear(); _wtables.clear()
                bump_weight_epoch(params=False)
                ver = (w._version, WEIGHT_EPOCH)
            _wplans[key] = pl
        _lib.check(_lib_().wdno_pack_split_weight(_p(wc), _p(amax), _p(pl.hi), _p(pl.lo), _p(pl.sc), k, c, kd, kh, kw, kp, cp8,
                                                  _wmode(kind), _stream()), 'pack_split_weight')
    pl.ver = ver
    pl.used = WEIGHT_EPOCH
    return pl.hi, pl.lo, pl.sc


ACT16 = os.environ.get('WDNO_ACT16', '0') == '1'
ZERO_BOX = True


class _ZeroBox(C.Structure):
    _fields_ = [('channels', C.c_int), ('d0', C.c_int), ('h0', C.c_int), ('w0', C.c_int)]


def set_zero_box(t, box):
    t._wdno_zero_box = (tuple(int(v) for v in box), t._version)
    return t


def zero_box_of(t):
    h = getattr(t, '_wdno_zero_box', None)
    return h[0] if h is not None and h[1] == t._version and ZERO_BOX else None


def carry_zero_box(dst, src):
    box = zero_box_of(src)
    return set_zero_box(dst, box) if box is not None else dst


def conv_fwd_h3(planes, shape4, w, pack, kind, bias_p, residual, ks, st, pd, kp, out=None, osp=None, ostride=(1, 1, 1), ooff=(0, 0, 0),
                amax_rec=None, zero_box=None, out16=False):
    xh, xl, sx = planes
    n, d, h, ww = shape4
    cp8 = xh.shape[-1]
    wh, wl, sw = split_weight(w, kind, cp8, kp, pack)
    if osp is None:
        osp = tuple(_out_size(a, k, s_, p_) for a, k, s_, p_ in zip((d, h, ww), ks, st, pd))
    out16 = bool(out16 and xl is None and out is None and residual is None)
    if out is None:
        y = torch.empty((n, *osp, kp), device=xh.device, dtype=torch.bfloat16 if out16 else torch.float32)
        g = _geom((n, d, h, ww), cp8, kp, ks, st, pd, osp)
    else:
        y = out
        g = _geom((n, d, h, ww), cp8, kp, ks, st, pd, osp, y_sp=tuple(out.shape[1:4]), ostride=ostride, ooff=ooff)
    flops = 2.0 * n * osp[0] * osp[1] * osp[2] * kp * ks[0] * ks[1] * ks[2] * cp8
    tap = (out is None and tuple(st) == (1, 1, 1) and tuple(osp) == (d, h, ww) and max(ks) <= 8 and
           ((ks[2] == 3 and cp8 % 32 == 0) or (ks[2] == 7 and cp8 % 16 == 0 and kp <= 64)))
    with _timed(_fwd_h3_kernel_name(n * osp[0] * osp[1] * osp[2], kp, ks, tap, cp8 if xl is not None else None), flops):
        zb = None
        if zero_box is not None and tap and ks[2] == 7:
            zb = _ZeroBox(*zero_box)
        if xl is None:
            if zb is not None or out16:
                _lib.check(_lib_().wdno_conv_fwd_bf16_ex(_p(xh), _p(wh), _p(bias_p), _p(residual), _p(y), int(out16), _p(amax_rec), C.byref(g),
                                                         None if zb is None else C.byref(zb), _stream()), 'conv_fwd_bf16_ex')
                return y
            _lib.check(_lib_().wdno_conv_fwd_bf16(_p(xh), _p(wh), _p(bias_p), _p(residual), _p(y), _p(amax_rec), C.byref(g), _stream()), 'conv_fwd_bf16')
            return y
        if zb is not None:
            _lib.check(_lib_().wdno_conv_fwd_f16x3_zbox(_p(xh), _p(xl), _p(sx), _p(wh), _p(wl), _p(sw), _p(bias_p), _p(residual), _p(y),
                                                        _p(amax_rec), C.byref(g), C.byref(zb), _stream()), 'conv_fwd_f16x3_zbox')
            return y
        key = (n, d, h, ww, cp8, kp, tuple(ks), tuple(osp)) if tap and ks[2] == 3 else None
        wsb = 0
        if key is not None:
            wsb = _split_ws_bytes.get(key)
            if wsb is None:
                wsb = _split_ws_bytes[key] = int(_lib_().wdno_conv_fwd_split_ws_bytes(C.byref(g)))
        if wsb:
            ws = torch.empty(wsb // 4, device=xh.device, dtype=torch.float32)
            _lib.check(_lib_().wdno_conv_fwd_f16x3_ws(_p(xh), _p(xl), _p(sx), _p(wh), _p(wl), _p(sw), _p(bias_p), _p(residual), _p(y),
                                                      _p(amax_rec), C.byref(g), _p(ws), wsb, _stream()), 'conv_fwd_f16x3_ws')
            return y
        _lib.check(_lib_().wdno_conv_fwd_f16x3_amax(_p(xh), _p(xl), _p(sx), _p(wh), _p(wl), _p(sw), _p(bias_p), _p(residual), _p(y),
                                                    _p(amax_rec), C.byref(g), _stream()), 'conv_fwd_f16x3')
    return y


_split_ws_bytes = {}


_pixel_tables = {}


def _fwd_h3_kernel_name(pixels, k, ks, tap=False, c=None):
    cdiv = lambda a, b: -(-a // b)
    tiles = cdiv(pixels, 128) * cdiv(k, 128) if k > 64 else cdiv(pixels, 256)
    small_tap = tap and ks[2] == 3 and cdiv(pixels, 64) * cdiv(k, 64) >= 64
    if (tiles >= 100 or small_tap) and max(ks) <= 8:
        cus = 256
        cost = lambda bm, bn, wgt: cdiv(cdiv(pixels, bm) * cdiv(k, bn), cus) * bm * bn * wgt
        shapes = [(256, 64, 1.04), (192, 64, 1.08)] if k <= 64 else [(128, 128, 1.0), (192, 128, 1.0), (256, 64, 1.04), (192, 64, 1.08)]
        best = shapes[0]
        for sh in shapes[1:]:
            if cost(*sh) < cost(*best):
                best = sh
        if tap and ks[2] == 3:
            c_best = cost(*best)
            if k > 64 and cost(160, 128, 1.02) < c_best:
                best, c_best = (160, 128, 1.02), cost(160, 128, 1.02)
            if cost(320, 64, 1.05) < c_best:
                best, c_best = (320, 64, 1.05), cost(320, 64, 1.05)
            if cost(128, 64, 1.15) < c_best:
                best, c_best = (128, 64, 1.15), cost(128, 64, 1.15)
            if cost(64, 64, 1.35) < c_best:
                best = (64, 64, 1.35)
            if best[:2] == (64, 64) and c is not None and c % 32 == 0 and k >= 128:
                t128, nst = cdiv(pixels, 128) * cdiv(k, 128), ks[0] * ks[1] * (c // 32)
                if t128 * 4 <= cus and nst % 4 == 0 and nst // 4 >= 8:
                    return 'conv_fwd_h3t_kernel<128,128>/4'
        if tap and _lp() and k > 64 and cdiv(pixels, 256) * cdiv(k, 128) >= 2 * cus:
            best = (256, 128)
        if tap and ks[2] == 7:
            best = (256, 64)
            if not _lp() and cdiv(pixels, 256) < cus and cdiv(pixels, 256) < cdiv(pixels, 192) <= cus:
                best = (192, 64)
        return f'conv_fwd_h3{"t" if tap else "d"}_kernel<{best[0]},{best[1]}>'
    return 'conv_fwd_h3_kernel<..,128>' if k > 64 else 'conv_fwd_h3_kernel<..,64>'


def _wgrad_h3_kernel_name(k, run, window=False):
    if window == 'stem':
        return 'conv_wgrad_h3s_kernel<64,352>'
    if window:
        return 'conv_wgrad_h3w_kernel<64,384>'
    cdiv = lambda a, b: -(-a // b)
    bn = 192 if cdiv(run, 192) * 192 <= cdiv(run, 128) * 128 else 128
    return f'conv_wgrad_h3d_kernel<{128 if k > 64 else 64},{bn}>'


FLAT_WGRAD = True
_FLAT_ARMED = False
DEFER_WGRAD_REDUCE = True
_WGRAD_PENDING = None
WGRAD_FLUSH_BYTES = int(os.environ.get('WDNO_WGRAD_FLUSH_MB', '0')) << 20
DEFER_ROW_SUMS = True
_ROWSUM_PENDING = []
_DEFERRED_DSTS = set()


def flush_wgrad_reduces():
    global _WGRAD_PENDING, _ROWSUM_PENDING
    pend, rows = _WGRAD_PENDING, _ROWSUM_PENDING
    if rows:
        _ROWSUM_PENDING = []
        ritems = (_lib.RowsSumItem * len(rows))(*[it for it, _ in rows])
        _lib.check(_lib_().wdno_rows_sum_multi(C.cast(ritems, C.c_void_p), len(rows), _stream()), 'rows_sum_multi')
        _DEFERRED_DSTS.update(int(it.out) for it, _ in rows)
    if not pend:
        return
    _WGRAD_PENDING = [] if _FLAT_ARMED else None
# ... 200 lines not shown
    if v is None or v.shape[0] == n:
        return v
    out = v.new_zeros((n,))
    out[:v.shape[0]] = v
    return out


LINEAR_MULTI_ROWS_MAX = 256
LINEAR_ROWS_MAX = 64


def _linear_rows_backward(ctx, gy):
    x, weight = ctx.saved_tensors
    _, _, _, k, c, cp, kp, has_bias, _, _, _ = ctx.meta
    gy = _chk(gy, 'grad')
    rows = x.shape[0]
    lib = _lib_()
    gx = gw = gb = None
    if ctx.needs_input_grad[0]:
        wt = _cached(weight, 'lin_t', 0, 0, lambda: weight.detach().t())
        gx = torch.empty((rows, cp), device=x.device, dtype=torch.float32)
        _lib.check(lib.wdno_linear_rows_fwd(_p(gy), kp, _p(wt), k, None, _p(gx), rows, k, c, cp, _stream()), 'linear_rows_dgrad')
    if ctx.needs_input_grad[1] or (has_bias and ctx.needs_input_grad[2]):
        gw = torch.empty((k, c), device=x.device, dtype=torch.float32)
        gb = torch.empty((k,), device=x.device, dtype=torch.float32) if has_bias else None
        _lib.check(lib.wdno_linear_rows_wgrad(_p(x), cp, _p(gy), kp, _p(gw), _p(gb), rows, c, k, _stream()), 'linear_rows_wgrad')
        gw = gw.reshape(weight.shape)
        if not ctx.needs_input_grad[1]:
            gw = None
        if not (has_bias and ctx.needs_input_grad[2]):
            gb = None
    return gx, gw, gb, None, None, None


class _Conv(torch.autograd.Function):

    @staticmethod
    def forward(ctx, x, weight, bias, residual, stride, padding, with_skip=False, grad_planes=False, to_norm=False):
        ctx.with_skip = with_skip
        ctx.to_norm = to_norm and grad_planes
        ctx.bias_ref = bias
        y = _Conv._forward(ctx, x, weight, bias, residual, stride, padding)
        if grad_planes and not ctx.rows and ctx.h3 and y.dim() in (4, 5) and residual is None:
            ks, st = ctx.meta[0], ctx.meta[1]
            n_, d_, h_, w_, _ = ctx.xshape
            if not ctx.needs_input_grad[0] or (st == (1, 1, 1) and _use_h3(n_ * d_ * h_ * w_, ctx.meta[6] * ks[0] * ks[1] * ks[2])):
                y._wdno_grad_planes = True
        if with_skip:
            return y, _alias_of(x)
        return y

    @staticmethod
    def _forward(ctx, x, weight, bias, residual, stride, padding):
        xrec = _known_amax(x)
        x_in = x
        ctx.x16 = x.dtype == torch.bfloat16
        if ctx.x16:
            if not (getattr(x, '_wdno_unwritten', False) and x.is_cuda):
                raise RuntimeError('wdno_amd: a bf16 tensor that is not a planes-only placeholder reached a convolution')
            x = x if x.is_contiguous() else x.contiguous()
        else:
            x = _chk(x, 'x')
        lead = None
        if x.dim() != 5:
            lead = x.shape[:-1]
            x5 = x.reshape(1, 1, 1, -1, x.shape[-1]) if x.dim() != 4 else x.unsqueeze(1)
        else:
            x5 = x
        w5 = _as5(weight)
        k, c = w5.shape[0], w5.shape[1]
        cp, kp = x5.shape[-1], pad4(k)
        assert cp == pad4(c), f'channel mismatch: tensor has {cp}, weight expects {c}'
        ks = tuple(w5.shape[2:])
        if x.dim() == 2 and x.shape[0] <= LINEAR_ROWS_MAX and weight.dim() == 2 and residual is None and c % 4 == 0 and k % 4 == 0:
            wc = weight.detach()
            wc = wc if wc.is_contiguous() else wc.contiguous()
            rows = x.shape[0]
            y = torch.empty((rows, kp), device=x.device, dtype=torch.float32)
            _lib.check(_lib_().wdno_linear_rows_fwd(_p(x), cp, _p(wc), c, _p(None if bias is None else bias.detach()), _p(y), rows, c, k, kp,
                                                    _stream()), 'linear_rows_fwd')
            ctx.save_for_backward(x, weight)
            ctx.h3 = False
            ctx.rows = True
            ctx.meta = (ks, stride, padding, k, c, cp, kp, bias is not None, False, lead, 2)
            return y
        ctx.rows = False
        with torch.no_grad():
            bias_p = _pad_vec(bias.detach() if bias is not None else None, kp)
        res5 = None
        if residual is not None:
            residual = _chk(residual, 'residual')
            res5 = residual
        osp_ = tuple(_out_size(a, kk, s_, p_) for a, kk, s_, p_ in zip(x5.shape[1:4], ks, stride, padding))
        h3 = _use_h3(x5.shape[0] * osp_[0] * osp_[1] * osp_[2], cp * ks[0] * ks[1] * ks[2])
        if getattr(x_in, '_wdno_unwritten', False):
            hp = getattr(x_in, '_wdno_planes', None)
            if not (h3 and hp is not None and hp[1] == x_in._version and hp[2] == CONV_MATH):
                raise RuntimeError('wdno_amd: a planes-only tensor reached a convolution that reads fp32')
        if h3:
            c8w = pad8(cp) + 8 if (ks[2] == 7 and kp <= 64 and tuple(stride) == (1, 1, 1) and pad8(cp) % 16) else None
            planes = split_f16_of(x_in, x5.reshape(-1, cp), xrec, c8w)
            yrec = _new_amax_record(x5.device)
            nx_, dx_, hx_, wx_ = x5.shape[:4]
            out16 = (ACT16 and _lp() and getattr(ctx, 'to_norm', False) and GRAD_PLANES and residual is None and x.dim() in (4, 5) and kp % 8 == 0
                     and kp // 8 <= 256 and (kp // 8) & (kp // 8 - 1) == 0
                     and (not ctx.needs_input_grad[0] or (tuple(stride) == (1, 1, 1) and _use_h3(nx_ * dx_ * hx_ * wx_, kp * ks[0] * ks[1] * ks[2]))))
            y = _leave_amax(conv_fwd_h3(planes, tuple(x5.shape[:4]), weight, pack_fwd, 'f', bias_p, res5, ks, stride, padding, kp,
                                        amax_rec=yrec, zero_box=zero_box_of(x_in) if x_in.dim() == 5 else None, out16=out16), yrec)
            ctx.save_for_backward(planes[0], planes[1], planes[2], weight)
        else:
            y = conv_fwd_raw(x5, pack_fwd(weight, cp, kp), bias_p, res5, ks, stride, padding, kp)
            ctx.save_for_backward(x5, weight)
        ctx.h3 = h3
        ctx.xshape = tuple(x5.shape)
        ctx.meta = (ks, stride, padding, k, c, cp, kp, bias is not None, residual is not None, lead, x.dim())
        if lead is not None:
            y = y.reshape(*lead, kp) if x.dim() != 4 else y.squeeze(1)
        return y

    @staticmethod
    def backward(ctx, gy, gskip=None):
        if ctx.rows:
            return _linear_rows_backward(ctx, gy) + (None, None, None)
        return _Conv._backward(ctx, gy, gskip) + (None, None, None)

    @staticmethod
    def _backward(ctx, gy, gskip):
        if ctx.h3:
            xh, xl, sx, weight = ctx.saved_tensors
            x5 = None
        else:
            x5, weight = ctx.saved_tensors
        ks, stride, padding, k, c, cp, kp, has_bias, has_res, lead, xdim = ctx.meta
        grec = _known_amax(gy)
        po = getattr(gy, '_wdno_planes_only', None)
        if po is not None and gy.dtype == torch.bfloat16:
            gy = gy if gy.is_contiguous() else gy.contiguous()
        else:
            gy = _chk(gy, 'grad')
        n, d, h, w, _ = ctx.xshape
        gyplanes = None
        gb_given = None
        if po is not None:
            if not (ctx.h3 and po[2] == gy._version and po[3] == CONV_MATH and not has_res):
                raise RuntimeError('wdno_amd: a planes-only gradient reached a convolution that cannot take it')
            gyplanes, gb_given = po[0], po[1]
        osp = tuple(_out_size(a, kk, s, p) for a, kk, s, p in zip((d, h, w), ks, stride, padding))
        gy5 = gy.reshape(n, *osp, kp)
        gx = gw = gb = gr = None
        want_gb = has_bias and ctx.needs_input_grad[2]
        will_split = (ctx.needs_input_grad[1] and ctx.h3) or (ctx.needs_input_grad[0] and stride == (1, 1, 1)
                                                              and _use_h3(n * d * h * w, kp * ks[0] * ks[1] * ks[2]))
        if po is not None:
            if not (will_split and (not ctx.needs_input_grad[0] or (stride == (1, 1, 1) and _use_h3(n * d * h * w, kp * ks[0] * ks[1] * ks[2])))):
                raise RuntimeError('wdno_amd: a planes-only gradient reached a convolution whose backward needs fp32 dy')
            if want_gb:
                gb = rows_sum_for_param(gb_given, getattr(ctx, 'bias_ref', None), k) if isinstance(gb_given, _RowsJob) else gb_given[:k].contiguous()
        elif want_gb and will_split:
            gyplanes, gbs = split_f16_colsum(gy5.reshape(-1, kp), grec, bias=getattr(ctx, 'bias_ref', None), k=k)
            gb = gbs[:k].contiguous()
        if ctx.needs_input_grad[0]:
            gs5 = None if gskip is None else _chk(gskip, 'skip gradient').reshape(n, d, h, w, cp)
            if stride == (1, 1, 1):
                pd = tuple(kk - 1 - p for kk, p in zip(ks, padding))
                if _use_h3(n * d * h * w, kp * ks[0] * ks[1] * ks[2]):
                    if gyplanes is None:
                        gyplanes = split_f16(gy5.reshape(-1, kp), grec)
                    drec = _new_amax_record(gy5.device)
                    gx5 = _leave_amax(conv_fwd_h3(gyplanes, tuple(gy5.shape[:4]), weight, lambda w_, c8_, k_: pack_dgrad(w_, k_, c8_), 'd', None, gs5,
                                                  ks, (1, 1, 1), pd, cp, amax_rec=drec, out16=getattr(ctx, 'x16', False) and gs5 is None), drec)
                else:
                    wd = pack_dgrad(weight, cp, kp)
                    gx5 = conv_fwd_raw(gy5, wd, None, gs5, ks, (1, 1, 1), pd, cp)
                gs5 = None
            elif ks == (1, 4, 4) and stride == (1, 2, 2) and padding == (0, 1, 1):
                oh_, ow_ = gy5.shape[2], gy5.shape[3]
                if ctx.h3 and _use_h3(n * d * oh_ * ow_, kp * 4) and _as5(weight).is_contiguous():
                    if gyplanes is None:
                        gyplanes = split_f16(gy5.reshape(-1, kp), grec)
                    drec = _new_amax_record(gy5.device)
                    gx5 = _leave_amax(conv_transpose_h3(gyplanes, tuple(gy5.shape[:4]), _as5(weight), None, cp, amax_rec=drec), drec)
                else:
                    wt = pack_transposed(_as5(weight), kp, cp)
                    gx5 = conv_transpose_raw(gy5, wt, None, cp)
            elif ks == (1, 2, 2) and stride == (1, 2, 2) and padding == (0, 0, 0):
                if ctx.h3 and _use_h3(n * d * gy5.shape[2] * gy5.shape[3], kp) and _as5(weight).is_contiguous() and PATCH_DGRAD_H3:
                    if gyplanes is None:
                        gyplanes = split_f16(gy5.reshape(-1, kp), grec)
                    drec = _new_amax_record(gy5.device)
                    gx5 = _leave_amax(_patch2_dgrad(gy5, weight, cp, kp, gyplanes, drec), drec)
                else:
                    gx5 = _patch2_dgrad(gy5, weight, cp, kp)
            else:
                raise RuntimeError(f'wdno_amd: unsupported convolution geometry for dgrad {ks} {stride} {padding}')
            if gs5 is not None:
                gx5 = gx5 + gs5
            if getattr(ctx, 'x16', False) and gx5.dtype != torch.bfloat16:
                gx5 = gx5.to(torch.bfloat16)
            gx = gx5
            if lead is not None:
                gx = gx5.reshape(*lead, cp) if xdim != 4 else gx5.squeeze(1)
        if ctx.needs_input_grad[1]:
            if ctx.h3:
                if gyplanes is None:
                    gyplanes = split_f16(gy5.reshape(-1, kp), grec)
                gw = conv_wgrad_h3((xh, xl, sx), (n, d, h, w), gyplanes, osp, ks, stride, padding, param_kc=(k, c),
                                   out=_flat_grad_out(weight, (k, c, *ks))).reshape(weight.shape)
            else:
                dwp = conv_wgrad_raw(x5, gy5, ks, stride, padding)
                gw = dwp[:, :, :k, :, :c].permute(2, 4, 0, 1, 3).reshape(weight.shape).contiguous()
        if want_gb and gb is None:
            gb = colsum(gy5.reshape(-1, kp))[:k].contiguous()
        if has_res and ctx.needs_input_grad[3]:
            gr = gy
        return gx, gw, gb, gr, None, None


def _patch2_dgrad(gy5, weight, cp, kp, gyplanes=None, amax_rec=None):
    n, d, oh, ow, _ = gy5.shape
    w5 = _as5(weight)
    gx = torch.empty((n, d, 2 * oh, 2 * ow, cp), device=gy5.device, dtype=torch.float32)
    lib = _lib_()
    if gyplanes is not None:
        for py in range(2):
            for px in range(2):
                conv_fwd_h3(gyplanes, (n, d, oh, ow), w5, None, f'q{py}{px}', None, None, (1, 1, 1), (1, 1, 1), (0, 0, 0), cp, out=gx,
                            osp=(d, oh, ow), ostride=(1, 2, 2), ooff=(0, py, px), amax_rec=amax_rec)
        return gx

    def build():
        wz = _padded(w5.detach(), kp, cp)
        return wz.permute(3, 4, 1, 0, 2).reshape(2, 2, cp, kp)
    wq = _cached(weight, 'p2', cp, kp, build)
    for py in range(2):
        for px in range(2):
            g = _geom((n, d, oh, ow), kp, cp, (1, 1, 1), (1, 1, 1), (0, 0, 0), (d, oh, ow),
                      y_sp=(d, 2 * oh, 2 * ow), ostride=(1, 2, 2), ooff=(0, py, px))
            _lib.check(lib.wdno_conv_fwd(_p(gy5), _p(wq[py, px]), None, None, _p(gx), C.byref(g), _stream()), 'patch2_dgrad')
    return gx


def conv_cl(x, weight, bias=None, stride=1, padding=0, residual=None, with_skip=False, grad_planes=False, to_norm=False):
    nd = weight.dim() - 2

    def trip(v, fill):
        if nd == 0:
            return (fill,) * 3
        v = (v,) * nd if isinstance(v, int) else tuple(v)
        return (fill,) * (3 - nd) + v
    return _Conv.apply(x, weight, bias, residual, trip(stride, 1), trip(padding, 0) if nd else (0, 0, 0), with_skip, grad_planes, to_norm)


def conv_cl_skip(x, weight, bias=None, stride=1, padding=0, grad_planes=False, to_norm=False):
    return conv_cl(x, weight, bias, stride, padding, None, True, grad_planes, to_norm)


class _ConvT(torch.autograd.Function):

    @staticmethod
    def forward(ctx, x, weight, bias):
        xrec = _known_amax(x)
        x = _chk(x, 'x')
        cin, cout = weight.shape[0], weight.shape[1]
        cin_p, cout_p = x.shape[-1], pad4(cout)
        assert cin_p == pad4(cin) and tuple(weight.shape[2:]) == (1, 4, 4)
        with torch.no_grad():
            bias_p = _pad_vec(bias.detach() if bias is not None else None, cout_p)
        n, d, h, w = x.shape[:4]
        h3 = _use_h3(n * d * h * w, 4 * cin_p) and cout_p % 8 == 0
        if h3:
            planes = split_f16(x.reshape(-1, cin_p), xrec)
            yrec = _new_amax_record(x.device)
            y = _leave_amax(conv_transpose_h3(planes, (n, d, h, w), weight, bias_p, cout_p, yrec), yrec)
            ctx.save_for_backward(weight, *planes)
        else:
            y = conv_transpose_raw(x, pack_transposed(weight, cin_p, cout_p), bias_p, cout_p)
            ctx.save_for_backward(x, weight)
        ctx.meta = (cin, cout, cin_p, cout_p, bias is not None, h3, (n, d, h, w))
        return y

    @staticmethod
    def backward(ctx, gy):
        cin, cout, cin_p, cout_p, has_bias, h3, xshape4 = ctx.meta
        grec = _known_amax(gy)
# ... 26 lines not shown

class _LinearItem(C.Structure):
    _fields_ = [('w', C.c_void_p), ('bias', C.c_void_p), ('K', C.c_int), ('k_start', C.c_int)]


_lin_tables = {}


def _linear_table(weights, biases, c):
    key = (tuple(w.data_ptr() for w in weights), tuple(0 if b is None else b.data_ptr() for b in biases), c)
    tab = _lin_tables.get(key)
    if tab is None:
        if len(_lin_tables) > 64:
            _lin_tables.clear()
        items = (_LinearItem * len(weights))()
        ks, start = [], 0
        for i, (w, b) in enumerate(zip(weights, biases)):
            items[i] = _LinearItem(w.data_ptr(), None if b is None else b.data_ptr(), w.shape[0], start)
            ks.append((w.shape[0], start))
            start += w.shape[0]
        dev = torch.frombuffer(bytearray(bytes(items)), dtype=torch.uint8).to(weights[0].device)
        tab = (dev, ks, start)
        _lin_tables[key] = tab
    return tab


class _LinearMulti(torch.autograd.Function):
    @staticmethod
    def forward(ctx, x, n, *wb):
        weights, biases = wb[:n], wb[n:]
        x = _chk(x, 'x')
        p, c = x.shape
        tab, ks, f = _linear_table(weights, biases, c)
        ybuf = torch.empty((p * f,), device=x.device, dtype=torch.float32)
        _lib.check(_lib_().wdno_linear_multi_fwd(_p(tab), len(ks), f, _p(x), _p(ybuf), p, c, _stream()), 'linear_multi_fwd')
        gbuf = torch.empty_like(ybuf)
        outs = []
        for k, start in ks:
            o = ybuf[p * start:p * (start + k)].view(p, k)
            o._wdno_grad_slot = gbuf[p * start:p * (start + k)].view(p, k)
            outs.append(o)
        ctx.save_for_backward(x, *[w for w in weights])
        ctx.meta = (tab, ks, f, p, c, [b is not None for b in biases])
        ctx.gbuf = gbuf
        return tuple(outs)

    @staticmethod
    def backward(ctx, *gys):
        x = ctx.saved_tensors[0]
        tab, ks, f, p, c, has_bias = ctx.meta
        gbuf = ctx.gbuf
        for (k, start), g in zip(ks, gys):
            slot = gbuf[p * start:p * (start + k)].view(p, k)
            if g is None:
                slot.zero_()
            elif g.data_ptr() != slot.data_ptr() or not g.is_contiguous():
                slot.copy_(g)
        lib = _lib_()
        n = len(ks)
        gx = None
        if ctx.needs_input_grad[0]:
            gx = torch.empty((p, c), device=x.device, dtype=torch.float32)
            nb = lib.wdno_linear_multi_dgrad_ws_bytes(f, p, c)
            ws = _ws(nb, x.device)
            _lib.check(lib.wdno_linear_multi_dgrad(_p(tab), n, f, _p(gbuf), _p(gx), p, c, _p(ws), nb, _stream()), 'linear_multi_dgrad')
        gw = torch.empty((f, c), device=x.device, dtype=torch.float32)
        gb = torch.empty((f,), device=x.device, dtype=torch.float32)
        _lib.check(lib.wdno_linear_multi_wgrad(_p(tab), n, f, _p(x), _p(gbuf), _p(gw), _p(gb), p, c, _stream()), 'linear_multi_wgrad')
        gws = tuple(gw[start:start + k] if ctx.needs_input_grad[2 + i] else None for i, (k, start) in enumerate(ks))
        gbs = tuple(gb[start:start + k] if hb and ctx.needs_input_grad[2 + n + i] else None for i, ((k, start), hb) in enumerate(zip(ks, has_bias)))
        return (gx, None) + gws + gbs


def linear_multi(x, layers):
    if not layers or x.dim() != 2 or x.shape[0] > LINEAR_MULTI_ROWS_MAX or x.shape[1] % 4 or x.shape[1] > 512 or x.dtype != torch.float32:
        return None
    ws = [l.weight for l in layers]
    if any(w.dim() != 2 or w.shape[1] != x.shape[1] or w.shape[0] % 4 or not w.is_contiguous() or w.dtype != torch.float32 for w in ws):
        return None
    bs = [l.bias for l in layers]
    return list(_LinearMulti.apply(x, len(ws), *ws, *bs))


def conv_transpose_h3(xplanes, shape4, weight, bias_p, cout_p, amax_rec=None):
    n, d, h, w = shape4
    y = torch.empty((n, d, 2 * h, 2 * w, cout_p), device=xplanes[0].device, dtype=torch.float32)
    for py in range(2):
        for px in range(2):
            conv_fwd_h3(xplanes, shape4, weight, pack_fwd, f'p{py}{px}', bias_p, None, (1, 2, 2), (1, 1, 1), (0, 1 - py, 1 - px),
                        cout_p, out=y, osp=(d, h, w), ostride=(1, 2, 2), ooff=(0, py, px), amax_rec=amax_rec)
    return y


def conv_transpose_cl(x, weight, bias=None):
    return _ConvT.apply(x, weight, bias)


def _claim_grad_slot(t):
    slot = getattr(t, '_wdno_grad_slot', None)
    if slot is not None:
        try:
            del t._wdno_grad_slot
        except AttributeError:
            pass
    return slot


class _GroupNormAct(torch.autograd.Function):
    @staticmethod
    def forward(ctx, x, gamma, beta, ss, groups, act_silu, eps, out_planes=False):
        x_in = x
        x = _chk_act(x, 'x')
        x16 = int(x.dtype == torch.bfloat16)
        n, c = x.shape[0], x.shape[-1]
        s = x.numel() // (n * c)
        lib = _lib_()
        nb = lib.wdno_groupnorm_ws_bytes(n, s, c, groups)
        ws = _ws(nb, x.device)
        stats = torch.empty((lib.wdno_groupnorm_stats_floats(n, c, groups),), device=x.device, dtype=torch.float32)
        ssc = None if ss is None else _chk(ss, 'scale_shift')
        ctx.ss_slot = _claim_grad_slot(ss) if ssc is ss else None
        c8_ = c // 8
        if out_planes and CONV_MATH in ('f16x3', 'bf16') and c % 8 == 0 and c8_ <= 256 and (c8_ & (c8_ - 1)) == 0:
            nbp = lib.wdno_groupnorm_fwd_planes_ws_bytes(n, s, c, groups)
            wsp = _ws(nbp, x.device)
            hi = torch.empty((n * s, c), device=x.device, dtype=torch.float16)
            lo = brec = scale = None
            if not _lp():
                lo = torch.empty((n * s, c), device=x.device, dtype=torch.float16)
                brec = _amax_slot(x.device)
                scale = brec[1:2]
            _lib.check(lib.wdno_groupnorm_act_fwd_planes_t(_p(x), x16, _p(gamma), _p(beta), _p(ssc), _p(hi), _p(lo), _p(scale), _p(stats), _p(brec),
                                                           n, s, c, groups, float(eps), int(act_silu), _p(wsp), nbp, _stream()), 'groupnorm_fwd_planes')
            ctx.save_for_backward(x, gamma, beta, ssc, stats)
            ctx.meta = (n, s, c, groups, int(act_silu))
            ctx.epoch = _param_epoch(gamma)
            ctx.grad_planes = GRAD_PLANES and getattr(x_in, '_wdno_grad_planes', False)
            y = torch.empty(x.shape, device=x.device, dtype=torch.bfloat16 if (x16 or (ACT16 and _lp())) else torch.float32)
            return _planes_only(y, (hi, lo, scale))
        y = torch.empty(x.shape, device=x.device, dtype=torch.float32)
        rec = _new_amax_record(x.device)
        _lib.check(lib.wdno_groupnorm_act_fwd_amax_t(_p(x), x16, _p(gamma), _p(beta), _p(ssc), _p(y), _p(stats), _p(rec), n, s, c, groups,
                                                     float(eps), int(act_silu), _p(ws), nb, _stream()), 'groupnorm_fwd')
        ctx.save_for_backward(x, gamma, beta, ssc, stats)
        ctx.meta = (n, s, c, groups, int(act_silu))
        ctx.epoch = _param_epoch(gamma)
        c8 = c // 8
        ctx.grad_planes = (GRAD_PLANES and getattr(x_in, '_wdno_grad_planes', False) and CONV_MATH in ('f16x3', 'bf16') and c % 8 == 0
                           and c8 <= 256 and (c8 & (c8 - 1)) == 0)
        return _leave_amax(y, rec)

    @staticmethod
    def backward(ctx, gy):
        x, gamma, beta, ss, stats = ctx.saved_tensors
        n, s, c, groups, act_silu = ctx.meta
        if getattr(ctx, 'epoch', None) not in (None, _param_epoch(gamma)):
            raise RuntimeError('wdno_amd GroupNorm backward: the parameters were updated (optimiser step / checkpoint load) between this forward and its backward')
        gy = _chk_act(gy, 'grad')
        x16, dy16 = int(x.dtype == torch.bfloat16), int(gy.dtype == torch.bfloat16)
        lib = _lib_()
        dgb = torch.empty((n, 2, c), device=x.device, dtype=torch.float32)
        dss = None if ss is None else (ctx.ss_slot if getattr(ctx, 'ss_slot', None) is not None else torch.empty_like(ss))
        if ctx.grad_planes and CONV_MATH in ('f16x3', 'bf16'):
            nb = lib.wdno_groupnorm_bwd_planes_ws_bytes(n, s, c, groups)
            ws = _ws(nb, x.device)
            hi = torch.empty((n * s, c), device=x.device, dtype=torch.float16)
            cs = torch.empty((c,), device=x.device, dtype=torch.float32)
            lo = rec = scale = None
            if not _lp():
                lo = torch.empty((n * s, c), device=x.device, dtype=torch.float16)
                rec = _amax_slot(x.device)
                scale = rec[1:2]
# ... 561 lines not shown
```

wdno_amd/smoke/video_diffusion_pytorch/video_diffusion_pytorch_conv3d.py:

```python
import math
from functools import partial

import torch
from torch import nn

from wdno_amd import ops


def exists(x):
    return x is not None


def default(val, d):
    if exists(val):
        return val
    return d() if callable(d) else d


def is_odd(n):
    return (n % 2) == 1


class RotaryEmbedding(nn.Module):

# ... 210 lines not shown
        rotary_emb = RotaryEmbedding(min(32, attn_dim_head))
        temporal_attn = lambda d: EinopsToAndFrom('b c f h w', 'b (h w) f c',
                                                  Attention(d, heads=attn_heads, dim_head=attn_dim_head, rotary_emb=rotary_emb))
        self.time_rel_pos_bias = RelativePositionBias(heads=attn_heads, max_distance=32)

        init_dim = default(init_dim, dim)
        assert is_odd(init_kernel_size)
        init_padding = init_kernel_size // 2
        self.init_conv = nn.Conv3d(channels, init_dim, (init_kernel_size,) * 3, padding=(init_padding,) * 3)
        self.init_temporal_attn = Residual(PreNorm(init_dim, temporal_attn(init_dim)))

        dims = [init_dim, *map(lambda m: dim * m, dim_mults)]
        in_out = list(zip(dims[:-1], dims[1:]))

        time_dim = dim * 4
        self.time_mlp = nn.Sequential(nn.Identity(), nn.Linear(dim, time_dim), nn.GELU(), nn.Linear(time_dim, time_dim))

        self.downs = nn.ModuleList([])
        self.ups = nn.ModuleList([])
        num_resolutions = len(in_out)
        block_klass = partial(ResnetBlock, groups=resnet_groups)
        block_klass_cond = partial(block_klass, time_emb_dim=time_dim)

        for ind, (dim_in, dim_out) in enumerate(in_out):
            is_last = ind >= (num_resolutions - 1)
            self.downs.append(nn.ModuleList([
                block_klass_cond(dim_in, dim_out),
                block_klass_cond(dim_out, dim_out),
                Residual(PreNorm(dim_out, SpatialLinearAttention(dim_out, heads=attn_heads))) if use_sparse_linear_attn else nn.Identity(),
                Residual(PreNorm(dim_out, temporal_attn(dim_out))),
                Downsample(dim_out) if not is_last else nn.Identity(),
            ]))

        mid_dim = dims[-1]
        self.mid_block1 = block_klass_cond(mid_dim, mid_dim)
        spatial_attn = EinopsToAndFrom('b c f h w', 'b f (h w) c', Attention(mid_dim, heads=attn_heads))
        self.mid_spatial_attn = Residual(PreNorm(mid_dim, spatial_attn))
        self.mid_temporal_attn = Residual(PreNorm(mid_dim, temporal_attn(mid_dim)))
        self.mid_block2 = block_klass_cond(mid_dim, mid_dim)

        for ind, (dim_in, dim_out) in enumerate(reversed(in_out)):
            is_last = ind >= (num_resolutions - 1)
            self.ups.append(nn.ModuleList([
                block_klass_cond(dim_out * 2, dim_in),
                block_klass_cond(dim_in, dim_in),
                Residual(PreNorm(dim_in, SpatialLinearAttention(dim_in, heads=attn_heads))) if use_sparse_linear_attn else nn.Identity(),
                Residual(PreNorm(dim_in, temporal_attn(dim_in))),
                Upsample(dim_in) if not is_last else nn.Identity(),
            ]))

        out_dim = default(out_dim, channels)
        self.out_dim = out_dim
        self.final_conv = nn.Sequential(block_klass(dim * 2, dim), nn.Conv3d(dim, out_dim, 1))

    def forward_with_cond_scale(self, *args, cond_scale=2., **kwargs):
        return self.forward(*args, null_cond_prob=0., **kwargs)

    def time_embedding(self, time):
        e = ops.sinusoidal_embedding(time, self.dim)
        e = ops.conv_cl(e, self.time_mlp[1].weight, self.time_mlp[1].bias)
        e = ops.gelu(e)
        return ops.conv_cl(e, self.time_mlp[3].weight, self.time_mlp[3].bias)

    def time_projections(self, t):
        blocks = getattr(self, '_time_blocks', None)
        if blocks is None:
            blocks = [b for lv in self.downs for b in lv[:2]] + [self.mid_block1, self.mid_block2] + [b for lv in self.ups for b in lv[:2]]
            object.__setattr__(self, '_time_blocks', blocks)
        out = ops.linear_multi(ops.silu_shared(t), [b.mlp[1] for b in blocks]) if all(exists(b.mlp) for b in blocks) else None
        return iter(out if out is not None else [None] * len(blocks))

    def forward(self, x, time, cond=None, null_cond_prob=0., focus_present_mask=None, prob_focus_present=0.):
        assert cond is None, 'cond must be None (has_cond is False on the WDNO path)'
        if prob_focus_present != 0.:
            raise NotImplementedError('prob_focus_present is always 0 on the WDNO path')
        b, f, c, h, w = x.shape
        x_api = x
        x = ops.nc_to_cl(x.reshape(b * f, c, h, w)).reshape(b, f, h, w, -1)
        ops.carry_zero_box(x, x_api)
        pos_bias = self.time_rel_pos_bias(f, device=x.device)

        x = ops.conv_cl(x, self.init_conv.weight, self.init_conv.bias, padding=self.init_conv.padding)
        x = self.init_temporal_attn(x, pos_bias=pos_bias)
        r = x
        t = self.time_embedding(time)
        ss = self.time_projections(t)

        hs = []
        for block1, block2, spatial_attn, temporal_attn, downsample in self.downs:
            x = block1(x, t, next(ss))
            x = block2(x, t, next(ss))
            if not isinstance(spatial_attn, nn.Identity):
                x = spatial_attn(x)
            x = temporal_attn(x, pos_bias=pos_bias, focus_present_mask=focus_present_mask)
            hs.append(x)
            if not isinstance(downsample, nn.Identity):
                x = ops.conv_cl(x, downsample.weight, downsample.bias, stride=(1, 2, 2), padding=(0, 1, 1))

        x = self.mid_block1(x, t, next(ss))
        x = self.mid_spatial_attn(x)
        x = self.mid_temporal_attn(x, pos_bias=pos_bias, focus_present_mask=focus_present_mask)
        x = self.mid_block2(x, t, next(ss))

        for block1, block2, spatial_attn, temporal_attn, upsample in self.ups:
            x = ops.concat_cl(x, hs.pop(), planes_only=ops.resnet_reads_planes(x.numel() // x.shape[-1], block1))
            x = block1(x, t, next(ss))
            x = block2(x, t, next(ss))
            if not isinstance(spatial_attn, nn.Identity):
                x = spatial_attn(x)
            x = temporal_attn(x, pos_bias=pos_bias, focus_present_mask=focus_present_mask)
            if not isinstance(upsample, nn.Identity):
                x = ops.conv_transpose_cl(x, upsample.weight, upsample.bias)

        x = ops.concat_cl(x, r, planes_only=ops.resnet_reads_planes(x.numel() // x.shape[-1], self.final_conv[0]))
        x = self.final_conv[0](x)
        x = ops.conv_cl(x, self.final_conv[1].weight, self.final_conv[1].bias)
        bb, ff, hh, ww, kp = x.shape
        return ops.cl_to_nc(x.reshape(bb * ff, hh, ww, kp), self.out_dim).reshape(bb, ff, self.out_dim, hh, ww)
```

Baseline: 32.20.

## Fuse concat-split and skip-add gradient junctions into conv backward epilogues

Adds a dual-output variant of the f16x3 convolution kernel that writes the two channel halves of its output to separate tensors, each with its own amax record. Conv data-gradient backward uses it so the concatenation backward gets its two halves directly, skipping the separate split kernel and the full-size intermediate. A fork autograd op marks skip-branch junctions, and the transposed-conv dgrad now folds the skip gradient in as a residual. The aim is fewer elementwise passes over memory in the U-Net backward. In exchange there is extra bookkeeping of tensor attributes and version checks, and a runtime error if an unwritten concat gradient is reached through another path.

```diff
diff --git a/include/wdno_hip.h b/include/wdno_hip.h
--- a/include/wdno_hip.h
+++ b/include/wdno_hip.h
@@ -94,6 +94,9 @@
                            const float* bias, const float* residual, float* y, float* amax_rec, const wdno_conv_geom* g,
                            void* ws, size_t ws_bytes, wdno_stream_t s);
 size_t wdno_conv_fwd_split_ws_bytes(const wdno_conv_geom* g);
+int wdno_conv_fwd_f16x3_dual(const void* xh, const void* xl, const float* sx, const void* wph, const void* wpl, const float* sw,
+                             const float* bias, const float* residual, float* ya, float* yb, int Ca, float* amax_rec_a, float* amax_rec_b,
+                             const wdno_conv_geom* g, wdno_stream_t s);
 size_t wdno_conv_wgrad_f16x3_ws_bytes(const wdno_conv_geom* g);
 int wdno_conv_pixel_table(void* table, const wdno_conv_geom* g, wdno_stream_t s);
 int wdno_conv_wgrad_f16x3(const void* xh, const void* xl, const float* sx, const void* dyh, const void* dyl, const float* sdy,
diff --git a/wdno_amd/_lib.py b/wdno_amd/_lib.py
--- a/wdno_amd/_lib.py
+++ b/wdno_amd/_lib.py
@@ -115,6 +115,7 @@
     'wdno_conv_fwd_bf16': (I, [P, P, P, P, P, P, PG, P]),
     'wdno_conv_fwd_f16x3_zbox': (I, [P, P, P, P, P, P, P, P, P, P, PG, P, P]),
     'wdno_conv_fwd_bf16_ex': (I, [P, P, P, P, P, I, P, PG, P, P]),
+    'wdno_conv_fwd_f16x3_dual': (I, [P, P, P, P, P, P, P, P, P, P, I, P, P, PG, P]),
     'wdno_conv_wgrad_bf16_param': (I, [P, P, P, P, I, I, P, Z, PG, P]),
     'wdno_conv_wgrad_ws_bytes': (Z, [PG]),
     'wdno_conv_wgrad': (I, [P, P, P, P, Z, PG, P]),
diff --git a/wdno_amd/csrc/conv_common.h b/wdno_amd/csrc/conv_common.h
--- a/wdno_amd/csrc/conv_common.h
+++ b/wdno_amd/csrc/conv_common.h
@@ -23,6 +23,9 @@
   size_t split_ws_bytes;
   int zb_blocks, zb_d, zb_h;
   int out_bf16;
+  float* y2;
+  float* amax_rec2;
+  int dual_ca;
 };
 
 __device__ __forceinline__ int xcd_swizzle(int bid, int nwg) {
@@ -71,6 +74,12 @@
   __builtin_amdgcn_s_waitcnt(0xc07f);
   asm volatile("s_barrier" : : : "memory");
 }
+struct ConvDst { float* base; int pitch; bool second; };
+__device__ __forceinline__ ConvDst conv_dst(const ConvP& p, float* y, int kb) {
+  if (p.y2 == nullptr) return {y, p.g.K, false};
+  if (kb < p.dual_ca) return {y, p.dual_ca, false};
+  return {p.y2 - p.dual_ca, p.g.K - p.dual_ca, true};
+}
 #endif
 static inline void fill_params(ConvP& p, const wdno_conv_geom* g) {
   p.g = *g;
@@ -81,6 +90,7 @@
   p.split_ws_bytes = 0;
   p.zb_blocks = 0; p.zb_d = 0; p.zb_h = 0;
   p.out_bf16 = 0;
+  p.y2 = nullptr; p.amax_rec2 = nullptr; p.dual_ca = 0;
   p.debug = wdno_debug_mode;
   p.R = g->kw * g->C;
   p.nchunk = cdiv(p.R, BK);
diff --git a/wdno_amd/csrc/conv_h3.hip b/wdno_amd/csrc/conv_h3.hip
--- a/wdno_amd/csrc/conv_h3.hip
+++ b/wdno_amd/csrc/conv_h3.hip
@@ -424,7 +424,7 @@
   }
 
   const float inv = LP ? 1.0f : 1.0f / (sx[0] * sw[0]);
-  float am = 0.f;
+  float am = 0.f, am2 = 0.f;
 #pragma unroll
   for (int a = 0; a < TM; ++a) {
 #pragma unroll
@@ -436,6 +436,7 @@
 #pragma unroll
       for (int b = 0; b < TN; ++b) {
         int kc = n0 + n_base + b * 32 + li;
+        const ConvDst dst = conv_dst(p, y, n0 + n_base + b * 32);
         if (kc < g.K) {
           float v = acc[a][b][e] * inv;
           if (p.ksplit > 1) {
@@ -449,13 +450,15 @@
           if (bias) v += bias[kc];
           if (res) v += res[yr * g.K + kc];
           if (LP && p.out_bf16) reinterpret_cast<unsigned short*>(y)[yr * g.K + kc] = bf16_rne(v);
-          else y[yr * g.K + kc] = v;
-          am = fmaxf(am, fabsf(v));
+          else dst.base[yr * dst.pitch + kc] = v;
+          if (dst.second) am2 = fmaxf(am2, fabsf(v));
+          else am = fmaxf(am, fabsf(v));
         }
       }
     }
   }
   if (p.amax_rec) wave_amax_emit(am, p.amax_rec, (int)blockIdx.x * 4 + wave);
+  if (p.amax_rec2) wave_amax_emit(am2, p.amax_rec2, (int)blockIdx.x * 4 + wave);
 }
 
 template <int BM, int BN, int WM, int WN, bool LP>
@@ -498,13 +501,18 @@
 template <bool LP>
 static int conv_fwd_16(const void* xh, const void* xl, const float* sx, const void* wph, const void* wpl, const float* sw,
                        const float* bias, const float* residual, float* y, float* amax_rec, const wdno_conv_geom* g, wdno_stream_t s,
-                       float* split_ws = nullptr, size_t split_ws_bytes = 0, const wdno_zero_box* zb = nullptr, int y_bf16 = 0) {
+                       float* split_ws = nullptr, size_t split_ws_bytes = 0, const wdno_zero_box* zb = nullptr, int y_bf16 = 0,
+                       float* y2 = nullptr, float* amax_rec2 = nullptr, int dual_ca = 0) {
   int rc = check_geom(g);
   if (rc) return rc;
   if (g->C & 7) return WDNO_EUNSUPPORTED;
   if (y_bf16 && (!LP || residual)) return WDNO_EUNSUPPORTED;
   ConvP p;
   fill_params(p, g);
+  if (y2) {
+    if (dual_ca <= 0 || dual_ca >= g->K || (dual_ca & 31) || y_bf16 || split_ws || !p.identity_out || y2 == y) return WDNO_EUNSUPPORTED;
+    p.y2 = y2; p.amax_rec2 = amax_rec2; p.dual_ca = dual_ca;
+  }
   p.out_bf16 = y_bf16 ? 1 : 0;
   if (zb) {
     if (zb->channels < 0 || zb->d0 < 0 || zb->h0 < 0 || zb->w0 < 0) return WDNO_EINVAL;
@@ -529,7 +537,10 @@
   if (K > 64) {
     if (blocks(128, 128) >= 512 || blocks(64, 128) < 2 * blocks(128, 128)) rc = launch_h3<128, 128, 2, 2, LP>(xh, xl, wph, wpl, sx, sw, bias, residual, y, p, st);
     else if (blocks(64, 128) < 200) {
-      if (blocks(64, 64) <= 384 && g->kd * g->kh >= 2 && p.nsteps >= 64 && p.identity_out && residual != y && !LP) p.ksplit = 2;
+      if (blocks(64, 64) <= 384 && g->kd * g->kh >= 2 && p.nsteps >= 64 && p.identity_out && residual != y && !LP) {
+        if (p.y2) return WDNO_EUNSUPPORTED;
+        p.ksplit = 2;
+      }
       rc = launch_h3<64, 64, 2, 2, LP>(xh, xl, wph, wpl, sx, sw, bias, residual, y, p, st);
     }
     else rc = launch_h3<64, 128, 1, 4, LP>(xh, xl, wph, wpl, sx, sw, bias, residual, y, p, st);
@@ -558,6 +569,14 @@
 extern "C" int wdno_conv_fwd_bf16_ex(const void* x16, const void* wp16, const float* bias, const float* residual, void* y, int y_bf16, float* amax_rec,
                                      const wdno_conv_geom* g, const wdno_zero_box* zb, wdno_stream_t s) {
   return conv_fwd_16<true>(x16, x16, nullptr, wp16, wp16, nullptr, bias, residual, (float*)y, amax_rec, g, s, nullptr, 0, zb, y_bf16);
+}
+extern "C" int wdno_conv_fwd_f16x3_dual(const void* xh, const void* xl, const float* sx, const void* wph, const void* wpl, const float* sw,
+                                        const float* bias, const float* residual, float* ya, float* yb, int Ca, float* amax_rec_a,
+                                        float* amax_rec_b, const wdno_conv_geom* g, wdno_stream_t s) {
+  if (!ya || !yb) return WDNO_EINVAL;
+  if (wdno_conv_fwd_split_ws_bytes(g)) return WDNO_EUNSUPPORTED;
+  if (xl == nullptr) return conv_fwd_16<true>(xh, xh, nullptr, wph, wph, nullptr, bias, residual, ya, amax_rec_a, g, s, nullptr, 0, nullptr, 0, yb, amax_rec_b, Ca);
+  return conv_fwd_16<false>(xh, xl, sx, wph, wpl, sw, bias, residual, ya, amax_rec_a, g, s, nullptr, 0, nullptr, 0, yb, amax_rec_b, Ca);
 }
 extern "C" size_t wdno_conv_fwd_split_ws_bytes(const wdno_conv_geom* g) {
   if (!g || check_geom(g) || (g->C & 7)) return 0;
diff --git a/wdno_amd/csrc/conv_h3d.hip b/wdno_amd/csrc/conv_h3d.hip
--- a/wdno_amd/csrc/conv_h3d.hip
+++ b/wdno_amd/csrc/conv_h3d.hip
@@ -147,7 +147,7 @@
     return;
   }
 
-  float am = 0.f;
+  float am = 0.f, am2 = 0.f;
   const int wm = wave / WN, wn = wave - wm * WN;
   const int li = lane & 31, hh = lane >> 5;
   const int m_base = wm * (TM * 32), n_base = wn * (TN * 32);
@@ -242,7 +242,6 @@
       const int64_t pm = m0 + m_base + a * 32 + li;
       if (pm >= p.P) continue;
       const int64_t yr = p.identity_out ? pm : out_row(g, pm);
-      float* yrow = y + yr * g.K;
       const float* rrow = res ? res + yr * g.K : nullptr;
       if (LP && p.out_bf16) {
         unsigned short* y16 = reinterpret_cast<unsigned short*>(y) + yr * g.K;
@@ -269,23 +268,29 @@
       }
 #pragma unroll
       for (int b = 0; b < TN; ++b) {
+        const ConvDst dst = conv_dst(p, y, n0 + n_base + b * 32);
+        float* yrow = dst.base + yr * dst.pitch;
+        float amb = 0.f;
 #pragma unroll
         for (int e4 = 0; e4 < 4; ++e4) {
           const int kc = n0 + n_base + b * 32 + 8 * e4 + 4 * hh;
           if (kc < g.K) {
             float4 v = make_float4(acc[a][b][4 * e4] * inv, acc[a][b][4 * e4 + 1] * inv, acc[a][b][4 * e4 + 2] * inv, acc[a][b][4 * e4 + 3] * inv);
-            if (bias) { const float4 t = *reinterpret_cast<const float4*>(bias + kc); v.x += t.x; v.y += t.y; v.z += t.z; v.w += t.w; }
-            if (rrow) { const float4 t = *reinterpret_cast<const float4*>(rrow + kc); v.x += t.x; v.y += t.y; v.z += t.z; v.w += t.w; }
+            if (bias) { const float4 tb = *reinterpret_cast<const float4*>(bias + kc); v.x += tb.x; v.y += tb.y; v.z += tb.z; v.w += tb.w; }
+            if (rrow) { const float4 tr = *reinterpret_cast<const float4*>(rrow + kc); v.x += tr.x; v.y += tr.y; v.z += tr.z; v.w += tr.w; }
             *reinterpret_cast<float4*>(yrow + kc) = v;
-            am = amax4(am, v);
+            amb = amax4(amb, v);
           }
         }
+        if (dst.second) am2 = fmaxf(am2, amb);
+        else am = fmaxf(am, amb);
       }
     }
     if (stamps) c_epi += __builtin_amdgcn_s_memtime() - e_begin;
   }
   if (stamps) am = sdbg == WDNO_DBG_STAMP_CYCLES ? (float)(__builtin_amdgcn_s_memtime() - c_begin) : sdbg == WDNO_DBG_STAMP_EPILOGUE ? (float)c_epi : (float)(__builtin_amdgcn_s_memrealtime() - r_begin);
   if (p.amax_rec) wave_amax_emit(am, p.amax_rec, (int)blockIdx.x * (WM * WN) + wave);
+  if (p.amax_rec2) wave_amax_emit(am2, p.amax_rec2, (int)blockIdx.x * (WM * WN) + wave);
 }
 
 template <int BM, int BN, int WM, int WN, int NS, bool LP>
diff --git a/wdno_amd/csrc/conv_h3t.hip b/wdno_amd/csrc/conv_h3t.hip
--- a/wdno_amd/csrc/conv_h3t.hip
+++ b/wdno_amd/csrc/conv_h3t.hip
@@ -242,7 +242,7 @@
     return;
   }
 
-  float am = 0.f;
+  float am = 0.f, am2 = 0.f;
   const int wm = wave / WN, wn = wave - wm * WN;
   const int li = lane & 31, hh = lane >> 5;
   const int m_base = wm * (TM * 32), n_base = wn * (TN * 32);
@@ -416,7 +416,6 @@
         }
         continue;
       }
-      float* yrow = y + yr * g.K;
       const float* rrow = res ? res + yr * g.K : nullptr;
       if (LP && p.out_bf16) {
         unsigned short* y16 = reinterpret_cast<unsigned short*>(y) + yr * g.K;
@@ -443,6 +442,9 @@
       }
 #pragma unroll
       for (int b = 0; b < TN; ++b) {
+        const ConvDst dst = conv_dst(p, y, n0 + n_base + b * 32);
+        float* yrow = dst.base + yr * dst.pitch;
+        float amb = 0.f;
 #pragma unroll
         for (int e4 = 0; e4 < 4; ++e4) {
           const int kc = n0 + n_base + b * 32 + 8 * e4 + 4 * hh;
@@ -451,15 +453,18 @@
             if (bias) { const float4 tb = *reinterpret_cast<const float4*>(bias + kc); v.x += tb.x; v.y += tb.y; v.z += tb.z; v.w += tb.w; }
             if (rrow) { const float4 tr = *reinterpret_cast<const float4*>(rrow + kc); v.x += tr.x; v.y += tr.y; v.z += tr.z; v.w += tr.w; }
             *reinterpret_cast<float4*>(yrow + kc) = v;
-            am = amax4(am, v);
+            amb = amax4(amb, v);
           }
         }
+        if (dst.second) am2 = fmaxf(am2, amb);
+        else am = fmaxf(am, amb);
       }
     }
     if (stamps) c_epi += __builtin_amdgcn_s_memtime() - e_begin;
   }
   if (stamps) am = sdbg == WDNO_DBG_STAMP_CYCLES ? (float)(__builtin_amdgcn_s_memtime() - c_begin) : sdbg == WDNO_DBG_STAMP_EPILOGUE ? (float)c_epi : (float)(__builtin_amdgcn_s_memrealtime() - r_begin);
   if (p.amax_rec) wave_amax_emit(am, p.amax_rec, (int)blockIdx.x * (WM * WN) + wave);
+  if (p.amax_rec2) wave_amax_emit(am2, p.amax_rec2, (int)blockIdx.x * (WM * WN) + wave);
 }
 
 __global__ __launch_bounds__(256) void conv_split_reduce_kernel(const float4* __restrict__ ws, int nruns, int64_t n4, int K4, const float* __restrict__ sx,
diff --git a/wdno_amd/ops.py b/wdno_amd/ops.py
--- a/wdno_amd/ops.py
+++ b/wdno_amd/ops.py
@@ -156,6 +156,7 @@
         p = a.numel() // ca
         out = torch.empty((*a.shape[:-1], ca + cb), device=a.device, dtype=torch.float32)
         ctx.ca, ctx.cb = ca, cb
+        ctx.cell = cell = {'ca': ca, 'cb': cb, 'issued': False} if FUSED_JUNCTIONS else None
         if (planes_only and PLANES_FWD and CONV_MATH in ('f16x3', 'bf16') and ca % 8 == 0 and cb % 8 == 0
                 and (_lp() or (ra is not None and rb is not None))):
             hi = torch.empty((p, ca + cb), device=a.device, dtype=torch.float16)
@@ -164,20 +165,54 @@
                 lo = torch.empty((p, ca + cb), device=a.device, dtype=torch.float16)
                 sc = torch.empty((1,), device=a.device, dtype=torch.float32)
             _lib.check(_lib_().wdno_concat2_cl_planes(_p(a), ca, _p(b), cb, _p(ra), _p(rb), _p(hi), _p(lo), _p(sc), p, _stream()), 'concat2_planes')
-            return _planes_only(out, (hi, lo, sc))
+            return _tag_concat(_planes_only(out, (hi, lo, sc)), cell)
         rec = _new_amax_record(a.device)
         _lib.check(_lib_().wdno_concat2_cl_amax(_p(a), ca, _p(b), cb, _p(out), _p(rec), p, _stream()), 'concat2_cl')
-        return _leave_amax(out, rec)
+        return _tag_concat(_leave_amax(out, rec), cell)
 
     @staticmethod
     def backward(ctx, g):
+        ca, cb = ctx.ca, ctx.cb
+        cell = getattr(ctx, 'cell', None)
+        h = getattr(g, '_wdno_halves', None)
+        if h is not None and h[2] == g._version and h[0].shape[-1] == ca and h[1].shape[-1] == cb:
+            cell['issued'] = False
+            return _reshaped(h[0], (*g.shape[:-1], ca)), _reshaped(h[1], (*g.shape[:-1], cb)), None
+        if cell is not None and cell['issued']:
+            raise RuntimeError('wdno_amd: the unwritten gradient of a concatenation reached its backward through another operation')
         g = _chk(g, 'grad')
-        ca, cb = ctx.ca, ctx.cb
         p = g.numel() // (ca + cb)
         ga = torch.empty((*g.shape[:-1], ca), device=g.device, dtype=torch.float32)
         gb = torch.empty((*g.shape[:-1], cb), device=g.device, dtype=torch.float32)
         _lib.check(_lib_().wdno_split2_cl(_p(g), _p(ga), ca, _p(gb), cb, p, _stream()), 'split2_cl')
         return ga, gb, None
+
+
+def _reshaped(t, shape):
+    if tuple(t.shape) == tuple(shape):
+        return t
+    v = t.view(shape)
+    h = getattr(t, '_wdno_amax', None)
+    if h is not None:
+        v._wdno_amax = h
+    return v
+
+
+def _tag_concat(out, cell):
+    if cell is not None:
+        out._wdno_concat = (cell, out._version)
+    return out
+
+
+def _claim_concat(t):
+    h = getattr(t, '_wdno_concat', None)
+    if h is None:
+        return None
+    try:
+        del t._wdno_concat
+    except AttributeError:
+        pass
+    return h[0] if h[1] == t._version and FUSED_JUNCTIONS else None
 
 
 def concat_cl(a, b, planes_only=False):
@@ -256,6 +291,27 @@
 
 def add(a, b):
     return _Add.apply(a, b)
+
+
+class _Fork(torch.autograd.Function):
+    @staticmethod
+    def forward(ctx, x):
+        ctx.set_materialize_grads(False)
+        return _alias_of(x), _alias_of(x)
+
+    @staticmethod
+    def backward(ctx, ga, gb):
+        if ga is None or gb is None:
+            return gb if ga is None else ga
+        ga, gb = _chk(ga, 'grad'), _chk(gb, 'skip gradient')
+        out = torch.empty_like(ga)
+        rec = _new_amax_record(ga.device)
+        _lib.check(_lib_().wdno_add_amax(_p(ga), _p(gb), _p(out), _p(rec), ga.numel(), _stream()), 'fork_bwd')
+        return _leave_amax(out, rec)
+
+
+def fork(x):
+    return _Fork.apply(x)
 
 
 def silu_shared(t):
@@ -380,6 +436,7 @@
 
 PLANES_FWD = True
 GRAD_PLANES = True
+FUSED_JUNCTIONS = True
 _CAPTURE = None
 
 
@@ -670,7 +727,9 @@
 
 
 def conv_fwd_h3(planes, shape4, w, pack, kind, bias_p, residual, ks, st, pd, kp, out=None, osp=None, ostride=(1, 1, 1), ooff=(0, 0, 0),
-                amax_rec=None, zero_box=None, out16=False):
+                amax_rec=None, zero_box=None, out16=False, dual=None):
+    if dual is not None:
+        amax_rec, amax_rec_b = amax_rec
     xh, xl, sx = planes
     n, d, h, ww = shape4
     cp8 = xh.shape[-1]
@@ -691,6 +750,22 @@
         zb = None
         if zero_box is not None and tap and ks[2] == 7:
             zb = _ZeroBox(*zero_box)
+        key = (n, d, h, ww, cp8, kp, tuple(ks), tuple(osp)) if tap and ks[2] == 3 and xl is not None else None
+        wsb = 0
+        if key is not None:
+            wsb = _split_ws_bytes.get(key)
+            if wsb is None:
+                wsb = _split_ws_bytes[key] = int(_lib_().wdno_conv_fwd_split_ws_bytes(C.byref(g)))
+        if dual is not None and out is None and not out16 and zb is None and not wsb and dual % 32 == 0 and 0 < dual < kp:
+            ya = torch.empty((n, *osp, dual), device=xh.device, dtype=torch.float32)
+            yb = torch.empty((n, *osp, kp - dual), device=xh.device, dtype=torch.float32)
+            rc = _lib_().wdno_conv_fwd_f16x3_dual(_p(xh), _p(xl), _p(sx), _p(wh), _p(wl), _p(sw), _p(bias_p), _p(residual), _p(ya), _p(yb), dual,
+                                                  _p(amax_rec), _p(amax_rec_b), C.byref(g), _stream())
+            if rc != -3:
+                _lib.check(rc, 'conv_fwd_f16x3_dual')
+                _poison(y)
+                y._wdno_halves = (_leave_amax(ya, amax_rec), _leave_amax(yb, amax_rec_b), y._version)
+                return y
         if xl is None:
             if zb is not None or out16:
                 _lib.check(_lib_().wdno_conv_fwd_bf16_ex(_p(xh), _p(wh), _p(bias_p), _p(residual), _p(y), int(out16), _p(amax_rec), C.byref(g),
@@ -702,12 +777,6 @@
             _lib.check(_lib_().wdno_conv_fwd_f16x3_zbox(_p(xh), _p(xl), _p(sx), _p(wh), _p(wl), _p(sw), _p(bias_p), _p(residual), _p(y),
                                                         _p(amax_rec), C.byref(g), C.byref(zb), _stream()), 'conv_fwd_f16x3_zbox')
             return y
-        key = (n, d, h, ww, cp8, kp, tuple(ks), tuple(osp)) if tap and ks[2] == 3 else None
-        wsb = 0
-        if key is not None:
-            wsb = _split_ws_bytes.get(key)
-            if wsb is None:
-                wsb = _split_ws_bytes[key] = int(_lib_().wdno_conv_fwd_split_ws_bytes(C.byref(g)))
         if wsb:
             ws = torch.empty(wsb // 4, device=xh.device, dtype=torch.float32)
             _lib.check(_lib_().wdno_conv_fwd_f16x3_ws(_p(xh), _p(xl), _p(sx), _p(wh), _p(wl), _p(sw), _p(bias_p), _p(residual), _p(y),
@@ -1074,6 +1143,7 @@
             ctx.save_for_backward(x, weight)
             ctx.h3 = False
             ctx.rows = True
+            ctx.concat = None
             ctx.meta = (ks, stride, padding, k, c, cp, kp, bias is not None, False, lead, 2)
             return y
         ctx.rows = False
@@ -1089,6 +1159,7 @@
             hp = getattr(x_in, '_wdno_planes', None)
             if not (h3 and hp is not None and hp[1] == x_in._version and hp[2] == CONV_MATH):
                 raise RuntimeError('wdno_amd: a planes-only tensor reached a convolution that reads fp32')
+        ctx.concat = _claim_concat(x_in) if h3 and not ctx.x16 else None
         if h3:
             c8w = pad8(cp) + 8 if (ks[2] == 7 and kp <= 64 and tuple(stride) == (1, 1, 1) and pad8(cp) % 16) else None
             planes = split_f16_of(x_in, x5.reshape(-1, cp), xrec, c8w)
@@ -1159,8 +1230,18 @@
                     if gyplanes is None:
                         gyplanes = split_f16(gy5.reshape(-1, kp), grec)
                     drec = _new_amax_record(gy5.device)
-                    gx5 = _leave_amax(conv_fwd_h3(gyplanes, tuple(gy5.shape[:4]), weight, lambda w_, c8_, k_: pack_dgrad(w_, k_, c8_), 'd', None, gs5,
-                                                  ks, (1, 1, 1), pd, cp, amax_rec=drec, out16=getattr(ctx, 'x16', False) and gs5 is None), drec)
+                    cell = getattr(ctx, 'concat', None)
+                    if cell is not None and cell['ca'] + cell['cb'] == cp and cell['ca'] % 32 == 0 and FUSED_JUNCTIONS:
+                        drec = (drec, _new_amax_record(gy5.device))
+                    else:
+                        cell = None
+                    gx5 = conv_fwd_h3(gyplanes, tuple(gy5.shape[:4]), weight, lambda w_, c8_, k_: pack_dgrad(w_, k_, c8_), 'd', None, gs5,
+                                      ks, (1, 1, 1), pd, cp, amax_rec=drec, out16=getattr(ctx, 'x16', False) and gs5 is None,
+                                      dual=None if cell is None else cell['ca'])
+                    if getattr(gx5, '_wdno_halves', None) is not None:
+                        cell['issued'] = True
+                    else:
+                        gx5 = _leave_amax(gx5, drec[0] if cell is not None else drec)
                 else:
                     wd = pack_dgrad(weight, cp, kp)
                     gx5 = conv_fwd_raw(gy5, wd, None, gs5, ks, (1, 1, 1), pd, cp)
@@ -1171,7 +1252,8 @@
                     if gyplanes is None:
                         gyplanes = split_f16(gy5.reshape(-1, kp), grec)
                     drec = _new_amax_record(gy5.device)
-                    gx5 = _leave_amax(conv_transpose_h3(gyplanes, tuple(gy5.shape[:4]), _as5(weight), None, cp, amax_rec=drec), drec)
+                    gx5 = _leave_amax(conv_transpose_h3(gyplanes, tuple(gy5.shape[:4]), _as5(weight), None, cp, amax_rec=drec, residual=gs5), drec)
+                    gs5 = None
                 else:
                     wt = pack_transposed(_as5(weight), kp, cp)
                     gx5 = conv_transpose_raw(gy5, wt, None, cp)
@@ -1192,6 +1274,9 @@
             gx = gx5
             if lead is not None:
                 gx = gx5.reshape(*lead, cp) if xdim != 4 else gx5.squeeze(1)
+                hv = getattr(gx5, '_wdno_halves', None)
+                if hv is not None:
+                    gx._wdno_halves = (hv[0], hv[1], gx._version)
         if ctx.needs_input_grad[1]:
             if ctx.h3:
                 if gyplanes is None:
@@ -1384,12 +1469,12 @@
     return list(_LinearMulti.apply(x, len(ws), *ws, *bs))
 
 
-def conv_transpose_h3(xplanes, shape4, weight, bias_p, cout_p, amax_rec=None):
+def conv_transpose_h3(xplanes, shape4, weight, bias_p, cout_p, amax_rec=None, residual=None):
     n, d, h, w = shape4
     y = torch.empty((n, d, 2 * h, 2 * w, cout_p), device=xplanes[0].device, dtype=torch.float32)
     for py in range(2):
         for px in range(2):
-            conv_fwd_h3(xplanes, shape4, weight, pack_fwd, f'p{py}{px}', bias_p, None, (1, 2, 2), (1, 1, 1), (0, 1 - py, 1 - px),
+            conv_fwd_h3(xplanes, shape4, weight, pack_fwd, f'p{py}{px}', bias_p, residual, (1, 2, 2), (1, 1, 1), (0, 1 - py, 1 - px),
                         cout_p, out=y, osp=(d, h, w), ostride=(1, 2, 2), ooff=(0, py, px), amax_rec=amax_rec)
     return y
 
diff --git a/wdno_amd/smoke/video_diffusion_pytorch/video_diffusion_pytorch_conv3d.py b/wdno_amd/smoke/video_diffusion_pytorch/video_diffusion_pytorch_conv3d.py
--- a/wdno_amd/smoke/video_diffusion_pytorch/video_diffusion_pytorch_conv3d.py
+++ b/wdno_amd/smoke/video_diffusion_pytorch/video_diffusion_pytorch_conv3d.py
@@ -316,7 +316,7 @@
 
         x = ops.conv_cl(x, self.init_conv.weight, self.init_conv.bias, padding=self.init_conv.padding)
         x = self.init_temporal_attn(x, pos_bias=pos_bias)
-        r = x
+        x, r = ops.fork(x) if ops.FUSED_JUNCTIONS else (x, x)
         t = self.time_embedding(time)
         ss = self.time_projections(t)
 
@@ -327,9 +327,16 @@
             if not isinstance(spatial_attn, nn.Identity):
                 x = spatial_attn(x)
             x = temporal_attn(x, pos_bias=pos_bias, focus_present_mask=focus_present_mask)
-            hs.append(x)
-            if not isinstance(downsample, nn.Identity):
-                x = ops.conv_cl(x, downsample.weight, downsample.bias, stride=(1, 2, 2), padding=(0, 1, 1))
+            if not ops.FUSED_JUNCTIONS:
+                hs.append(x)
+                if not isinstance(downsample, nn.Identity):
+                    x = ops.conv_cl(x, downsample.weight, downsample.bias, stride=(1, 2, 2), padding=(0, 1, 1))
+            elif not isinstance(downsample, nn.Identity):
+                x, xs = ops.conv_cl_skip(x, downsample.weight, downsample.bias, stride=(1, 2, 2), padding=(0, 1, 1))
+                hs.append(xs)
+            else:
+                x, xs = ops.fork(x)
+                hs.append(xs)
 
         x = self.mid_block1(x, t, next(ss))
         x = self.mid_spatial_attn(x)
```

Result: no change. 32.36 (median of 6 runs) (+0.5%).
